# johannesulf/nautilus

Measured on AMD Instinct MI355X. Metric: effective posterior samples/sec + |dlogZ| vs analytic, 50-dim Gaussian, higher is better.
Workload: dtype f64

## Files before the change

include/nautilus_hip.h:

```cpp
#ifndef NAUTILUS_HIP_H
#define NAUTILUS_HIP_H

#include <stdint.h>

#ifdef __cplusplus
extern "C" {
#endif

#define NB_ABI_VERSION 6

typedef struct nb_bound nb_bound;
typedef struct nb_boundlist nb_boundlist;

typedef struct {
  int32_t n_ell;
  const int32_t* idx_ell;
  const double* c;
  const double* B;
  const double* B_inv;
  int32_t free_dims;
} nb_member_desc;

typedef struct {
  int32_t n_networks;
  const double* mean;
  const double* scale;
  const double* const* coefs;
  const double* const* intercepts;
} nb_mlp_desc;

typedef struct {
  nb_member_desc ellipsoid;
  const nb_mlp_desc* mlp;
  double score_predict_min;
  double radius2;
} nb_neural_desc;

typedef struct {
  int32_t n_dim;
  int32_t n_members;
  const nb_member_desc* members;
  const double* log_v_all;
  int32_t unit_cube;
  int32_t n_neural;
  const nb_neural_desc* neural;
  int32_t n_periodic;
  const int32_t* periodic;
  const double* centers;
} nb_bound_desc;

int nb_abi_version(void);
const char* nb_last_error(void);

int nb_bound_create(const nb_bound_desc* desc, nb_bound** out);
int nb_bound_destroy(nb_bound* bound);
int64_t nb_bound_nbytes(const nb_bound* bound);

int nb_boundlist_create(nb_bound* const* bounds, int32_t n, nb_boundlist** out);
int nb_boundlist_destroy(nb_boundlist* list);

int nb_contains(const nb_bound* bound, const double* x_dev, int64_t n,
                uint8_t* mask_dev, void* stream);

int nb_contains_any(const nb_boundlist* list, const double* x_dev, int64_t n,
                    uint8_t* mask_dev, void* stream);

int nb_first_containing(const nb_boundlist* list, const double* x_dev,
                        int64_t n, int32_t* idx_dev, void* stream);

int nb_member_count(const nb_bound* bound, const double* x_dev, int64_t n,
                    uint8_t* count_dev, void* stream);

int nb_neural_score(const nb_bound* bound, const double* x_dev, int64_t n,
                    double* out_dev, void* stream);

int nb_propose(const nb_bound* bound, uint64_t seed, uint64_t offset,
               int64_t n, double* x_dev, void* stream);

int nb_accept(const nb_bound* bound, uint64_t seed, uint64_t offset,
              const double* x_dev, int64_t n, uint8_t* flags_dev,
              void* stream);

int64_t nb_compact_scratch_bytes(int64_t n);
int nb_compact_rows(const double* x_dev, const uint8_t* flags_dev,
                    uint8_t mask, uint8_t flip, int64_t n, int32_t n_dim,
                    double* out_dev, int64_t* src_idx_dev, int64_t* counts_dev,
                    void* scratch_dev, void* stream);

int nb_shell_stats(const double* log_l_dev, int64_t n, double threshold,
                   double* out_dev, void* scratch_dev, void* stream);
int64_t nb_shell_stats_scratch_bytes(int64_t n);

int nb_live_append(const double* log_l_dev, int64_t n, const double* thr_dev,
                   double* pool_dev, int32_t* pool_n_dev, int32_t capacity,
                   int32_t* overflow_dev, void* stream);
int nb_live_select(const double* pool_dev, const int32_t* pool_n_dev,
                   int32_t capacity, int32_t k, double* pool_out_dev,
                   int32_t* pool_out_n_dev, double* thr_dev, double* stats_dev,
                   void* stream);
int nb_live_stats(const double* log_l_dev, int64_t n, const double* thr_dev,
                  double* out_dev, void* stream);

typedef struct nb_trainer nb_trainer;
int nb_trainer_create(int32_t n_dim, int32_t n_networks, int64_t n_rows,
                      const double* x_dev, const double* y_dev,
                      const double* const* coefs_host,
                      const double* const* intercepts_host,
                      nb_trainer** out);
int nb_trainer_create_fleet(int32_t n_dim, int32_t n_networks,
                            const int64_t* n_rows_of,
                            const double* const* x_dev_of,
                            const double* const* y_dev_of,
                            const double* const* coefs_host,
                            const double* const* intercepts_host,
                            nb_trainer** out);
#define NB_TRAIN_MAX_BATCH 4096
int nb_trainer_set_hparams(nb_trainer* t, double lr, double beta1,
                           double beta2, double epsilon, int32_t batch,
                           int32_t max_iter, int32_t n_iter_no_change,
                           double tol);
int nb_trainer_run(nb_trainer* t, const int32_t* perm_dev, int32_t n_epochs,
                   int32_t* status_host, void* stream);
int nb_trainer_run_fleet(nb_trainer* t, const int32_t* const* perm_dev_of,
                         int32_t n_epochs, int32_t* status_host, void* stream);
int nb_trainer_status(nb_trainer* t, int32_t* status_host, void* stream);
int nb_trainer_run_async(nb_trainer* t, const int32_t* const* perm_dev_of,
                         int32_t n_epochs, void* stream, int64_t* ticket);
int nb_trainer_wait(nb_trainer* t, int64_t ticket, int32_t* status_host);
int nb_host_shuffle_epochs(int32_t n_streams, uint32_t* const* key_of,
                           int32_t* pos, const int64_t* n_of, int32_t n_epochs,
                           int32_t* const* order_of, int32_t* const* out_of);
int nb_trainer_loss_curve(nb_trainer* t, int32_t net, double* out_host,
                          int32_t max_len);
int nb_trainer_weights(nb_trainer* t, int32_t net, double* const* coefs_host,
                       double* const* intercepts_host);
int nb_trainer_destroy(nb_trainer* t);

int nb_philox_uniform(uint64_t seed, uint64_t offset, uint32_t block,
                      uint32_t tag, int64_t n, double* u_dev, void* stream);

int nb_set_eval_counters(uint64_t* counters_dev);

int nb_mfma_f64_peak(int32_t iters, double* tflops_host);

int64_t nb_mvee_weights_work_doubles(int64_t n, int32_t n_dim,
                                     int32_t n_batch);
int nb_mvee_weights(const double* x_dev, int64_t n, int32_t n_dim,
                    int32_t n_max, int32_t n_batch, double* u_dev,
                    double* work_dev, void* stream);

int64_t nb_whiten_work_doubles(int64_t n, int32_t n_dim);
int nb_whiten(const double* x_dev, int64_t n, int32_t n_dim, double* xw_dev,
              double* mean_dev, double* sd_dev, double* w_dev,
              double* work_dev, void* stream);

int64_t nb_mvee_work_doubles(int32_t n_problems, int64_t n_points_max,
                             int32_t n_dim, int32_t n_batch);
int nb_mvee_khachiyan(int32_t n_problems, const double* const* xs_dev,
                      const int64_t* n_points, int32_t n_dim, int32_t n_max,
                      int32_t n_batch, double* const* u_dev, double* work_dev,
                      void* stream);

int64_t nb_moments_work_doubles(int64_t n, int32_t n_dim);
int nb_weighted_moments(const double* x_dev, const double* w_dev, int64_t n,
                        int32_t n_dim, double scale, double* out_dev,
                        double* work_dev, void* stream);

int64_t nb_quadform_work_doubles(void);
int nb_quadform_max(const double* x_dev, int64_t n, int32_t n_dim,
                    const double* p_dev, double* out_dev, double* work_dev,
                    void* stream);

int nb_ellipsoid_transform(const nb_bound* bound, const double* x_dev,
                           int64_t n, double* y_dev, void* stream);

int nb_standardize(const double* x_dev, int64_t n, int32_t n_dim,
                   double* mean_dev, double* scale_dev, double* out_dev,
                   void* stream);

int nb_prior_transform(const double* u_dev, int64_t n, int32_t n_dim,
                       const uint8_t* kind, const double* loc,
                       const double* scale, double* out_dev, void* stream);

typedef struct nb_prior_table nb_prior_table;
#define NB_PRIOR_ROW_MAJOR 0
#define NB_PRIOR_COLUMN_MAJOR 1
#define NB_PRIOR_LOG_SPACE 35.0
#define NB_PRIOR_TRUNCNORM_MAX 1e150
int nb_prior_table_create(int32_t n_dim, const uint8_t* kind,
                          const double* loc, const double* scale,
                          const double* shape0, const double* shape1,
                          int32_t n_keys, const int32_t* key_column,
                          const double* key_value, nb_prior_table** out);
int nb_prior_table_destroy(nb_prior_table* table);
int nb_prior_table_transform(const nb_prior_table* table, const double* u_dev,
                             int64_t n, int32_t layout, double* out_dev,
                             void* stream);

int nb_loglike_rosenbrock(const double* u_dev, int64_t n, int32_t n_dim,
                          double lo, double hi, double a, double* out_dev,
                          void* stream);
int nb_loglike_funnel(const double* u_dev, int64_t n, int32_t n_dim, double mu,
                      double sigma0, double k, double c, double* out_dev,
                      void* stream);


int64_t nb_list_eval_work_bytes(const nb_boundlist* list, int64_t n);
int nb_list_eval(const nb_boundlist* list, int32_t mode, const double* x_dev,
                 int64_t n, uint8_t* st_dev, int32_t* first_dev, void* work_dev,
                 int64_t work_bytes, void* stream);
int64_t nb_accept_staged_work_bytes(const nb_bound* bound, int64_t n);
int nb_accept_staged(const nb_bound* bound, uint64_t seed, uint64_t offset,
                     const double* x_dev, int64_t n, uint8_t* flags_dev,
                     void* work_dev, int64_t work_bytes, int64_t* totals_offset,
                     void* stream);
int nb_neural_score_rows(const nb_bound* bound, int32_t m, int32_t recentre,
                         const double* x_dev, const int64_t* idx_dev,
                         int64_t n, double* out_dev, void* stream);

int64_t nb_gmm_out_doubles(int32_t n_dim);
int64_t nb_gmm_scratch_doubles(int64_t n, int32_t n_dim);
int64_t nb_gmm_work_doubles(int64_t n, int32_t n_dim, int32_t n_init);
int64_t nb_gmm_logp_offset(int32_t n_dim);
int nb_gmm_fit(const double* x_dev, int64_t n, int32_t n_dim, int32_t n_init,
               uint64_t seed, double tol, double reg_covar, int32_t max_iter,
               const int32_t* init_labels_dev, double* out_dev,
               double* scratch_dev, void* stream);
int nb_gmm_set_max_wgs(int32_t max_wgs);

int nb_phase_shift(double* x_dev, int64_t n, int32_t n_dim, int32_t n_periodic,
                   const int32_t* periodic, const double* centers,
                   int32_t inverse, void* stream);

#define NB_COMM_ID_BYTES 128
typedef struct nb_comm nb_comm;
int nb_comm_unique_id(uint8_t* id_out );
int nb_comm_init(int32_t rank, int32_t n_ranks, const uint8_t* id,
                 nb_comm** out);
int nb_comm_destroy(nb_comm* comm);
uint64_t nb_comm_rank_key(uint64_t seed, int32_t rank);
int nb_comm_allgather_f64(nb_comm* comm, const double* send_dev, int64_t count,
                          double* recv_dev ,
                          void* stream);
int nb_comm_allreduce_i64(nb_comm* comm, int64_t* buf_dev ,
                          int64_t count, void* stream);

int nb_ellipsoid_contains_stream(const nb_bound* bound, const double* x_dev,
                                 int64_t n, uint8_t* mask_dev, void* stream);

#ifdef __cplusplus
}
#endif
#endif
```

nautilus_amd/_lib.py:

```python

import ctypes as C
import os

_HERE = os.path.dirname(os.path.abspath(__file__))
LIB_PATH = os.environ.get('NAUTILUS_HIP_LIB') or os.path.join(
    _HERE, 'lib', 'libnautilus_hip.so')

ABI_VERSION = 6

c_double_p = C.POINTER(C.c_double)
c_int32_p = C.POINTER(C.c_int32)


class MemberDesc(C.Structure):
    _fields_ = [('n_ell', C.c_int32), ('idx_ell', c_int32_p),
                ('c', c_double_p), ('B', c_double_p), ('B_inv', c_double_p),
                ('free_dims', C.c_int32)]


class MlpDesc(C.Structure):
    _fields_ = [('n_networks', C.c_int32), ('mean', c_double_p),
                ('scale', c_double_p), ('coefs', C.POINTER(c_double_p)),
                ('intercepts', C.POINTER(c_double_p))]


class NeuralDesc(C.Structure):
    _fields_ = [('ellipsoid', MemberDesc), ('mlp', C.POINTER(MlpDesc)),
                ('score_predict_min', C.c_double), ('radius2', C.c_double)]


class BoundDesc(C.Structure):
    _fields_ = [('n_dim', C.c_int32), ('n_members', C.c_int32),
                ('members', C.POINTER(MemberDesc)), ('log_v_all', c_double_p),
                ('unit_cube', C.c_int32), ('n_neural', C.c_int32),
                ('neural', C.POINTER(NeuralDesc)),
                ('n_periodic', C.c_int32), ('periodic', c_int32_p),
                ('centers', c_double_p)]


_SIGNATURES = {
    'nb_abi_version': (C.c_int, []),
    'nb_last_error': (C.c_char_p, []),
    'nb_bound_create': (C.c_int, [C.POINTER(BoundDesc),
                                  C.POINTER(C.c_void_p)]),
    'nb_bound_destroy': (C.c_int, [C.c_void_p]),
    'nb_bound_nbytes': (C.c_int64, [C.c_void_p]),
    'nb_boundlist_create': (C.c_int, [C.POINTER(C.c_void_p), C.c_int32,
                                      C.POINTER(C.c_void_p)]),
    'nb_boundlist_destroy': (C.c_int, [C.c_void_p]),
    'nb_contains': (C.c_int, [C.c_void_p, C.c_void_p, C.c_int64, C.c_void_p,
                              C.c_void_p]),
    'nb_contains_any': (C.c_int, [C.c_void_p, C.c_void_p, C.c_int64,
                                  C.c_void_p, C.c_void_p]),
    'nb_first_containing': (C.c_int, [C.c_void_p, C.c_void_p, C.c_int64,
                                      C.c_void_p, C.c_void_p]),
    'nb_member_count': (C.c_int, [C.c_void_p, C.c_void_p, C.c_int64,
                                  C.c_void_p, C.c_void_p]),
    'nb_neural_score': (C.c_int, [C.c_void_p, C.c_void_p, C.c_int64,
                                  C.c_void_p, C.c_void_p]),
    'nb_propose': (C.c_int, [C.c_void_p, C.c_uint64, C.c_uint64, C.c_int64,
                             C.c_void_p, C.c_void_p]),
    'nb_accept': (C.c_int, [C.c_void_p, C.c_uint64, C.c_uint64, C.c_void_p,
                            C.c_int64, C.c_void_p, C.c_void_p]),
    'nb_compact_scratch_bytes': (C.c_int64, [C.c_int64]),
    'nb_compact_rows': (C.c_int, [C.c_void_p, C.c_void_p, C.c_uint8,
                                  C.c_uint8, C.c_int64, C.c_int32, C.c_void_p,
                                  C.c_void_p, C.c_void_p, C.c_void_p,
                                  C.c_void_p]),
    'nb_shell_stats': (C.c_int, [C.c_void_p, C.c_int64, C.c_double,
                                 C.c_void_p, C.c_void_p, C.c_void_p]),
    'nb_shell_stats_scratch_bytes': (C.c_int64, [C.c_int64]),
    'nb_trainer_create': (C.c_int, [C.c_int32, C.c_int32, C.c_int64,
                                    C.c_void_p, C.c_void_p,
                                    C.POINTER(c_double_p),
                                    C.POINTER(c_double_p),
                                    C.POINTER(C.c_void_p)]),
    'nb_trainer_create_fleet': (C.c_int, [C.c_int32, C.c_int32, C.c_void_p,
                                          C.c_void_p, C.c_void_p, C.c_void_p,
                                          C.c_void_p, C.c_void_p]),
    'nb_trainer_run_fleet': (C.c_int, [C.c_void_p, C.c_void_p, C.c_int32,
                                       C.c_void_p, C.c_void_p]),
    'nb_trainer_set_hparams': (C.c_int, [C.c_void_p, C.c_double, C.c_double,
                                         C.c_double, C.c_double, C.c_int32,
                                         C.c_int32, C.c_int32, C.c_double]),
    'nb_trainer_run': (C.c_int, [C.c_void_p, C.c_void_p, C.c_int32,
                                 c_int32_p, C.c_void_p]),
    'nb_trainer_status': (C.c_int, [C.c_void_p, c_int32_p, C.c_void_p]),
    'nb_trainer_run_async': (C.c_int, [C.c_void_p, C.c_void_p, C.c_int32,
                                       C.c_void_p, C.POINTER(C.c_int64)]),
    'nb_trainer_wait': (C.c_int, [C.c_void_p, C.c_int64, c_int32_p]),
    'nb_host_shuffle_epochs': (C.c_int, [C.c_int32, C.c_void_p, c_int32_p,
                                         C.c_void_p, C.c_int32, C.c_void_p,
                                         C.c_void_p]),
    'nb_trainer_loss_curve': (C.c_int, [C.c_void_p, C.c_int32, c_double_p,
                                        C.c_int32]),
    'nb_trainer_weights': (C.c_int, [C.c_void_p, C.c_int32,
                                     C.POINTER(c_double_p),
                                     C.POINTER(c_double_p)]),
    'nb_trainer_destroy': (C.c_int, [C.c_void_p]),
    'nb_philox_uniform': (C.c_int, [C.c_uint64, C.c_uint64, C.c_uint32,
                                    C.c_uint32, C.c_int64, C.c_void_p,
                                    C.c_void_p]),
    'nb_set_eval_counters': (C.c_int, [C.c_void_p]),
    'nb_mfma_f64_peak': (C.c_int, [C.c_int32, c_double_p]),
    'nb_mvee_weights': (C.c_int, [C.c_void_p, C.c_int64, C.c_int32, C.c_int32,
                                  C.c_int32, C.c_void_p, C.c_void_p,
                                  C.c_void_p]),
    'nb_mvee_weights_work_doubles': (C.c_int64, [C.c_int64, C.c_int32,
                                                 C.c_int32]),
    'nb_mvee_work_doubles': (C.c_int64, [C.c_int32, C.c_int64, C.c_int32,
                                         C.c_int32]),
    'nb_mvee_khachiyan': (C.c_int, [C.c_int32, C.POINTER(C.c_void_p),
                                    C.POINTER(C.c_int64), C.c_int32,
                                    C.c_int32, C.c_int32,
                                    C.POINTER(C.c_void_p), C.c_void_p,
                                    C.c_void_p]),
    'nb_whiten_work_doubles': (C.c_int64, [C.c_int64, C.c_int32]),
    'nb_whiten': (C.c_int, [C.c_void_p, C.c_int64, C.c_int32, C.c_void_p,
                            C.c_void_p, C.c_void_p, C.c_void_p, C.c_void_p,
                            C.c_void_p]),
    'nb_moments_work_doubles': (C.c_int64, [C.c_int64, C.c_int32]),
    'nb_weighted_moments': (C.c_int, [C.c_void_p, C.c_void_p, C.c_int64,
                                      C.c_int32, C.c_double, C.c_void_p,
                                      C.c_void_p, C.c_void_p]),
    'nb_quadform_work_doubles': (C.c_int64, []),
    'nb_quadform_max': (C.c_int, [C.c_void_p, C.c_int64, C.c_int32,
                                  C.c_void_p, C.c_void_p, C.c_void_p,
                                  C.c_void_p]),
    'nb_ellipsoid_transform': (C.c_int, [C.c_void_p, C.c_void_p, C.c_int64,
                                         C.c_void_p, C.c_void_p]),
    'nb_standardize': (C.c_int, [C.c_void_p, C.c_int64, C.c_int32, C.c_void_p,
                                 C.c_void_p, C.c_void_p, C.c_void_p]),
    'nb_prior_transform': (C.c_int, [C.c_void_p, C.c_int64, C.c_int32,
                                     C.c_void_p, c_double_p, c_double_p,
                                     C.c_void_p, C.c_void_p]),
    'nb_prior_table_create': (C.c_int, [C.c_int32, C.c_void_p, c_double_p,
                                        c_double_p, c_double_p, c_double_p,
                                        C.c_int32, c_int32_p, c_double_p,
                                        C.POINTER(C.c_void_p)]),
    'nb_prior_table_destroy': (C.c_int, [C.c_void_p]),
    'nb_prior_table_transform': (C.c_int, [C.c_void_p, C.c_void_p, C.c_int64,
                                           C.c_int32, C.c_void_p, C.c_void_p]),
    'nb_loglike_rosenbrock': (C.c_int, [C.c_void_p, C.c_int64, C.c_int32,
                                        C.c_double, C.c_double, C.c_double,
                                        C.c_void_p, C.c_void_p]),
    'nb_loglike_funnel': (C.c_int, [C.c_void_p, C.c_int64, C.c_int32,
                                    C.c_double, C.c_double, C.c_double,
                                    C.c_double, C.c_void_p, C.c_void_p]),
    'nb_live_append': (C.c_int, [C.c_void_p, C.c_int64, C.c_void_p,
                                 C.c_void_p, C.c_void_p, C.c_int32,
                                 C.c_void_p, C.c_void_p]),
    'nb_live_select': (C.c_int, [C.c_void_p, C.c_void_p, C.c_int32, C.c_int32,
                                 C.c_void_p, C.c_void_p, C.c_void_p,
                                 C.c_void_p, C.c_void_p]),
    'nb_live_stats': (C.c_int, [C.c_void_p, C.c_int64, C.c_void_p,
                                C.c_void_p, C.c_void_p]),
    'nb_comm_unique_id': (C.c_int, [C.c_void_p]),
    'nb_comm_init': (C.c_int, [C.c_int32, C.c_int32, C.c_void_p,
                               C.POINTER(C.c_void_p)]),
    'nb_comm_destroy': (C.c_int, [C.c_void_p]),
    'nb_comm_rank_key': (C.c_uint64, [C.c_uint64, C.c_int32]),
    'nb_comm_allgather_f64': (C.c_int, [C.c_void_p, C.c_void_p, C.c_int64,
                                        C.c_void_p, C.c_void_p]),
    'nb_comm_allreduce_i64': (C.c_int, [C.c_void_p, C.c_void_p, C.c_int64,
                                        C.c_void_p]),
    'nb_list_eval_work_bytes': (C.c_int64, [C.c_void_p, C.c_int64]),
    'nb_list_eval': (C.c_int, [C.c_void_p, C.c_int32, C.c_void_p, C.c_int64,
                               C.c_void_p, C.c_void_p, C.c_void_p, C.c_int64,
                               C.c_void_p]),
    'nb_accept_staged_work_bytes': (C.c_int64, [C.c_void_p, C.c_int64]),
    'nb_accept_staged': (C.c_int, [C.c_void_p, C.c_uint64, C.c_uint64,
                                   C.c_void_p, C.c_int64, C.c_void_p,
                                   C.c_void_p, C.c_int64,
                                   C.POINTER(C.c_int64), C.c_void_p]),
    'nb_neural_score_rows': (C.c_int, [C.c_void_p, C.c_int32, C.c_int32,
                                       C.c_void_p, C.c_void_p, C.c_int64,
                                       C.c_void_p, C.c_void_p]),
    'nb_gmm_out_doubles': (C.c_int64, [C.c_int32]),
    'nb_gmm_scratch_doubles': (C.c_int64, [C.c_int64, C.c_int32]),
    'nb_gmm_work_doubles': (C.c_int64, [C.c_int64, C.c_int32, C.c_int32]),
    'nb_gmm_logp_offset': (C.c_int64, [C.c_int32]),
    'nb_gmm_fit': (C.c_int, [C.c_void_p, C.c_int64, C.c_int32, C.c_int32,
                             C.c_uint64, C.c_double, C.c_double, C.c_int32,
                             C.c_void_p, C.c_void_p, C.c_void_p, C.c_void_p]),
    'nb_gmm_set_max_wgs': (C.c_int, [C.c_int32]),
    'nb_phase_shift': (C.c_int, [C.c_void_p, C.c_int64, C.c_int32, C.c_int32,
                                 c_int32_p, c_double_p, C.c_int32,
                                 C.c_void_p]),
    'nb_ellipsoid_contains_stream': (C.c_int, [C.c_void_p, C.c_void_p,
                                               C.c_int64, C.c_void_p,
                                               C.c_void_p]),
}

_lib = None


def load():
    global _lib
    if _lib is not None:
        return _lib
    try:
        import torch
    except ImportError:
        pass
    if not os.path.exists(LIB_PATH):
        raise RuntimeError(
            'nautilus_amd: HIP library %s not found; run `make` (hipcc, '
            'gfx950).  There is no CPU fallback.' % LIB_PATH)
    lib = C.CDLL(LIB_PATH)
    for name, (res, args) in _SIGNATURES.items():
        fn = getattr(lib, name)
        fn.restype = res
        fn.argtypes = args
    if lib.nb_abi_version() != ABI_VERSION:
        raise RuntimeError(
            'nautilus_amd: %s has ABI version %d, this package binds version '
            '%d (rebuild with `make`)' % (LIB_PATH, lib.nb_abi_version(),
                                          ABI_VERSION))
    _lib = lib
    return lib


def exported_symbols():
    return sorted(_SIGNATURES)


ERR_ARG, ERR_HIP, ERR_UNSUPPORTED = 1, 2, 3


class NativeError(RuntimeError):

    def __init__(self, code, message):
        super().__init__('nautilus_hip: ' + message)
        self.code = code


def check(status):
    if status != 0:
        raise NativeError(status, load().nb_last_error().decode(
            'utf-8', 'replace'))
```

nautilus_amd/csrc/nb_api.hip:

```cpp
#include "nb_common.h"
#include "../../include/nautilus_hip.h"

#include <cmath>
#include <cstdarg>
#include <cstdio>
#include <csignal>
#include <cstring>
#include <ctime>
#include <execinfo.h>
#include <limits>
#include <unistd.h>
#include <string>
#include <vector>

bool nb_eval_fast_eligible(int n_dim, int K, int M, int E, bool sample);
int nb_launch_eval_fast(const double* blob_dev, int n_dim, bool sample, int m,
                        int recentre, const double* x, const long long* idx,
                        long long n,
                        unsigned char* out_u8, double* out_f64,
                        unsigned long long seed, unsigned long long offset,
                        hipStream_t stream);
int nb_launch_cand(int dt, int n_dim, const double* const* blobs_dev,
                   const int* group_base_dev, int nb, int n_groups, int b_off,
                   int g_off, int accumulate, int mode, const double* x,
                   long long n, unsigned char* st, int* first, int* work,
                   unsigned long long seed, unsigned long long offset,
                   int** dense_out, int** totals_out, long long* n_pad_out,
                   hipStream_t stream);
long long nb_cand_work_bytes(int dt, int mode, long long n, int n_groups);
int nb_launch_eval_fast_batch(const double* blob0_dev, int n_dim, int recentre,
                              const double* x, const void* groups_dev,
                              int n_groups, const int* totals_dev,
                              const int* dense_dev, long long n_pad,
                              long long n_upper, int out_mode,
                              unsigned char* st, int* first,
                              hipStream_t stream);
int nb_launch_eval(int dt, const double* const* blobs_dev, int nb, int mode,
                   const double* x, long long n, unsigned char* out_u8,
                   int* out_i32, double* out_f64, unsigned long long seed,
                   unsigned long long offset, hipStream_t stream);
void nb_eval_set_counters(unsigned long long* dev);
int nb_launch_draw(const double* blob_dev, int n_dim, unsigned long long seed,
                   unsigned long long offset, long long n, double* x_out,
                   hipStream_t stream);
long long nb_compact_chunks(long long n);
int nb_launch_compact(const double* x, const unsigned char* flags,
                      unsigned char mask, unsigned char flip, long long n,
                      int n_dim, double* out,
                      long long* src_idx, long long* counts,
                      long long* chunk_counts, hipStream_t stream);
int nb_lse_blocks(long long n);
int nb_launch_shell_stats(const double* log_l, long long n, double threshold,
                          double* out, double* partial, hipStream_t stream);
int nb_launch_philox(unsigned long long seed, unsigned long long offset,
                     unsigned block, unsigned tag, long long n, double* u,
                     hipStream_t stream);
int nb_run_mfma_peak(int iters, double* tflops);
int nb_launch_mvee_batch(int n_problems, const double* const* xs,
                         const long long* n, int d, int n_max, int n_batch,
                         double* const* u, double* work, hipStream_t stream);
long long nb_mvee_work_doubles_impl(int n_problems, long long n_max, int d,
                                    int n_batch);
int nb_launch_moments(const double* x, const double* w, long long n, int d,
                      double scale, double* out, double* work,
                      hipStream_t stream);
long long nb_moments_work_doubles_impl(long long n, int d);
int nb_launch_quadform_max(const double* x, long long n, int d,
                           const double* p_dev, double* out, double* work,
                           hipStream_t stream);
long long nb_quadform_work_doubles_impl();
int nb_launch_live_append(const double* ll, long long n, const double* thr,
                          double* pool, int* pool_n, int cap, int* overflow,
                          hipStream_t stream);
int nb_launch_live_select(const double* pool, const int* pool_n, int cap,
                          int k, double* out, int* out_n, double* thr,
                          double* stats, hipStream_t stream);
int nb_launch_live_stats(const double* ll, long long n, const double* thr,
                         double* out, hipStream_t stream);
int nb_launch_rosenbrock(const double* u, long long n, int d, double lo,
                         double hi, double a, double* out, hipStream_t stream);
int nb_launch_funnel(const double* u, long long n, int d, double mu, double s0,
                     double k, double c, double* out, hipStream_t stream);
long long nb_whiten_work_doubles_impl(long long n, int d);
int nb_launch_whiten(const double* x, long long n, int d, double* xw,
                     double* mean, double* sd, double* w, double* work,
                     hipStream_t stream);
int nb_launch_transform(const double* ell_block, int dt, int n_dim,
                        const double* x, long long n, double* y,
                        hipStream_t stream);
int nb_launch_standardize(const double* x, long long n, int d, double* mean,
                          double* scale, double* out, hipStream_t stream);
int nb_launch_prior(const double* u, long long n, int d,
                    const unsigned char* kind, const double* loc,
                    const double* scale, double* out, hipStream_t stream);
int nb_launch_prior_table(const double* u, long long n, int d,
                          const double* par, const unsigned char* kind,
                          int n_keys, const int* key_column,
                          const double* key_value, int column_major,
                          int level, double* out, hipStream_t stream);
long long nb_gmm_out_stride_impl(int d);
long long nb_gmm_scratch_stride_impl(long long n, int d);
long long nb_gmm_work_doubles_impl(long long n, int d, int n_init);
long long nb_gmm_logp_offset_impl(long long n, int d);
int nb_gmm_set_cap_impl(int max_wgs);
int nb_launch_gmm(const double* x, long long n, int d, int n_init,
                  unsigned long long seed, double tol, double reg, int max_iter,
                  const int* init_labels, double* out, double* scratch,
                  hipStream_t stream);
int nb_launch_phase_shift(double* x, long long n, int n_dim, const double* s,
                          const unsigned char* on, int inverse,
                          hipStream_t stream);
int nb_launch_ell_stream(const double* cvec, const double* binv, int n_dim,
                         const double* x, long long n, unsigned char* mask,
                         hipStream_t stream);

static thread_local std::string g_error;

void nb_set_error(const char* fmt, ...) {
  char buf[1024];
  va_list ap;
  va_start(ap, fmt);
  vsnprintf(buf, sizeof buf, fmt, ap);
  va_end(ap);
  g_error = buf;
}

struct nb_bound {
  double* blob_dev = nullptr;
  const double** self_list_dev = nullptr;
  FastGroup* groups_dev = nullptr;
  int* group_base_dev = nullptr;
  int n_groups = 0;
  int64_t off_shift = 0, neural_stride = 0;
  int64_t n_doubles = 0;
  int n_dim = 0, dt = 0, K = 0, M = 0, E = 0;
  bool single_full_ellipsoid = false;
  int64_t off_stream = 0;
  int64_t off_members = 0, off_neural = 0;
};

static inline int64_t nb_hdr_host_off_members(const nb_bound* b) {
  return b->off_members;
}

struct nb_boundlist {
  const double** ptrs_dev = nullptr;
  int n = 0, dt = 0, n_dim = 0;
  int blocks_single = 0;
  FastGroup* groups_dev = nullptr;
  int* group_base_dev = nullptr;
  std::vector<int> group_base;
  int n_groups = 0;
  const double* blob0 = nullptr;
};

static void nb_append_groups(const nb_bound* b, int pos,
                             std::vector<FastGroup>& out) {
  if (b->E < 1) return;
  for (int m = 0; m < b->M; ++m) {
    FastGroup g;
    g.nb = b->blob_dev + b->off_neural + (int64_t)m * b->neural_stride;
    g.shift = b->off_shift != 0 ? b->blob_dev + b->off_shift : nullptr;
    g.E = b->E;
    g.b = pos;
    out.push_back(g);
  }
}

namespace {

const double INF = std::numeric_limits<double>::infinity();

inline void put_i64(std::vector<double>& buf, size_t at, int64_t v) {
  std::memcpy(&buf[at], &v, sizeof v);
}

inline int slot_of_feature(int f) {
  const int j = f >> 3, r = f & 7;
  const int lg = r >> 1, o = r & 1;
  return 4 * (2 * j + o) + lg;
}

bool fill_ell_block(std::vector<double>& buf, size_t at, int n_dim, int dt,
                    const nb_member_desc& m, bool is_neural) {
  const int dp = 16 * dt;
  if (m.n_ell < 0 || m.n_ell > n_dim) {
    nb_set_error("member n_ell=%d out of range for n_dim=%d", m.n_ell, n_dim);
    return false;
  }
  put_i64(buf, at, m.n_ell);
  double* lo = &buf[at + 2];
  double* hi = lo + dp;
  double* c = hi + dp;
  double* tiles = c + dp;
  std::vector<int> idx(m.n_ell);
  std::vector<char> is_ell(n_dim, 0);
  for (int i = 0; i < m.n_ell; ++i) {
    idx[i] = m.idx_ell ? m.idx_ell[i] : i;
    if (idx[i] < 0 || idx[i] >= n_dim || (i > 0 && idx[i] <= idx[i - 1])) {
      nb_set_error("idx_ell must be strictly increasing within [0, n_dim)");
      return false;
    }
    is_ell[idx[i]] = 1;
  }
  bool any_box = false;
  for (int f = 0; f < dp; ++f) {
    const bool boxed = f < n_dim && !is_ell[f] && !m.free_dims && !is_neural;
    const int sl = slot_of_feature(f);
    lo[sl] = boxed ? 0.0 : -INF;
    hi[sl] = boxed ? 1.0 : INF;
    c[sl] = 0.0;
    any_box |= boxed;
  }
  put_i64(buf, at + 1, any_box ? 1 : 0);
  for (int i = 0; i < m.n_ell; ++i) c[slot_of_feature(idx[i])] = m.c[i];
  for (int i = 0; i < m.n_ell; ++i) {
    for (int j = 0; j < m.n_ell; ++j) {
      const double v = m.B_inv[(size_t)i * m.n_ell + j];
      if (j > i) {
        if (v != 0.0) {
          nb_set_error("B_inv must be lower triangular (basic.py:308-309)");
          return false;
        }
        continue;
      }
      const int h = idx[i], k = idx[j];
      const int sl = slot_of_feature(k);
      const int ks = sl >> 2, lgk = sl & 3;
      tiles[((size_t)(ks >> 2) * dt + (h >> 4)) * NB_TILE + (ks & 3) * 64 +
            lgk * 16 + (h & 15)] = v;
    }
  }
  return true;
}

void put_weight(double* tiles, int ht_n, int k, int h, double v) {
  tiles[((size_t)(k >> 4) * ht_n + (h >> 4)) * NB_TILE + (k & 15) * 16 +
        (h & 15)] = v;
}

void fill_net(double* net, int n_dim, int kt1, const double* const* coefs,
              const double* const* intercepts) {
  double* w1 = net;
  double* w2 = w1 + (size_t)kt1 * NB_HT1 * NB_TILE;
  double* w3 = w2 + (size_t)NB_HT1 * NB_HT2 * NB_TILE;
  double* w4 = w3 + (size_t)NB_HT2 * NB_HT3 * NB_TILE;
  for (int k = 0; k < n_dim; ++k)
    for (int h = 0; h < NB_H1; ++h)
      put_weight(w1, NB_HT1, k, h, coefs[0][(size_t)k * NB_H1 + h]);
  for (int h = 0; h < NB_H1; ++h)
    put_weight(w1, NB_HT1, n_dim, h, intercepts[0][h]);
  for (int k = 0; k < NB_H1; ++k)
    for (int h = 0; h < NB_H2; ++h)
      put_weight(w2, NB_HT2, k, h, coefs[1][(size_t)k * NB_H2 + h]);
  for (int h = 0; h < NB_H2; ++h)
    put_weight(w2, NB_HT2, NB_H1, h, intercepts[1][h]);
  for (int k = 0; k < NB_H2; ++k)
    for (int h = 0; h < NB_H3; ++h)
      put_weight(w3, NB_HT3, k, h, coefs[2][(size_t)k * NB_H3 + h]);
  for (int h = 0; h < NB_H3; ++h)
    put_weight(w3, NB_HT3, NB_H2, h, intercepts[2][h]);
  for (int k = 0; k < NB_H3; ++k) put_weight(w4, 1, k, 0, coefs[3][k]);
  put_weight(w4, 1, NB_H3, 0, intercepts[3][0]);
}

inline hipStream_t as_stream(void* s) { return (hipStream_t)s; }

}

extern "C" {

int nb_abi_version(void) { return NB_ABI_VERSION; }

const char* nb_last_error(void) { return g_error.c_str(); }

int nb_bound_create(const nb_bound_desc* d, nb_bound** out) {
  if (d == nullptr || out == nullptr) {
    nb_set_error("null argument");
    return NB_ERR_ARG;
  }
  const int n_dim = d->n_dim;
  if (n_dim < 1 || n_dim > 16 * NB_MAX_DT) {
    nb_set_error("n_dim=%d unsupported (1..%d)", n_dim, 16 * NB_MAX_DT);
    return NB_ERR_UNSUPPORTED;
  }
  const int dt = (n_dim + 15) / 16, dp = 16 * dt;
  const int K = d->n_members, M = d->n_neural;
  if (K < 0 || M < 0 || (K > 0 && d->members == nullptr) ||
      (M > 0 && d->neural == nullptr)) {
    nb_set_error("inconsistent member / neural counts");
    return NB_ERR_ARG;
  }
  int E = 0;
  for (int m = 0; m < M; ++m) {
    const int e = d->neural[m].mlp ? d->neural[m].mlp->n_networks : 0;
    if (m > 0 && e != E) {
      nb_set_error("all neural bounds must have the same number of networks");
      return NB_ERR_ARG;
    }
    E = e;
    if (d->neural[m].ellipsoid.n_ell != n_dim) {
      nb_set_error("NeuralBound ellipsoid must span all dimensions");
      return NB_ERR_ARG;
    }
  }
  const int kt1 = (n_dim + 1 + 15) / 16;
  const int64_t ell_size = nb_ell_block_size(dt);
  const int64_t net_stride = (int64_t)nb_net_tiles(kt1) * NB_TILE;
  const int64_t neural_stride = ell_size + 2 + 2 * dp + (int64_t)E * net_stride;
  const int64_t draw_stride = 2 + 4 * dp + (int64_t)dp * (dp + 1) / 2 + 16;

  int64_t off = NB_HDR;
  const int64_t off_cdf = off; off += ((K > 0 ? K : 1) + 1) / 2 * 2;
  const int64_t off_ulo = off; off += dp;
  const int64_t off_uhi = off; off += dp;
  const int64_t off_members = off; off += (int64_t)K * ell_size;
  const int64_t off_neural = off; off += (int64_t)M * neural_stride;
  const int64_t off_draw = off; off += (int64_t)K * draw_stride;
  const bool single_full = (K == 1 && M == 0 && !d->unit_cube &&
                            d->members[0].n_ell == n_dim);
  const int64_t off_stream = off;
  if (single_full) off += dp + (int64_t)dt * (dt + 1) / 2 * NB_TILE;
  if (d->n_periodic < 0 || d->n_periodic > n_dim ||
      (d->n_periodic > 0 && (d->periodic == nullptr || d->centers == nullptr))) {
    nb_set_error("bad periodic description");
    return NB_ERR_ARG;
  }
  const int64_t off_shift = off;
  if (d->n_periodic > 0) off += 2 * dp;
  const int64_t total = off;

  std::vector<double> buf((size_t)total, 0.0);
  put_i64(buf, NB_H_NDIM, n_dim);
  put_i64(buf, NB_H_DT, dt);
  put_i64(buf, NB_H_K, K);
  put_i64(buf, NB_H_USECUBE, d->unit_cube ? 1 : 0);
  put_i64(buf, NB_H_M, M);
  put_i64(buf, NB_H_E, E);
  put_i64(buf, NB_H_OFF_CDF, off_cdf);
  put_i64(buf, NB_H_OFF_ULO, off_ulo);
  put_i64(buf, NB_H_OFF_UHI, off_uhi);
  put_i64(buf, NB_H_OFF_MEMBERS, off_members);
  put_i64(buf, NB_H_ELL_STRIDE, ell_size);
  put_i64(buf, NB_H_OFF_NEURAL, off_neural);
  put_i64(buf, NB_H_NEURAL_STRIDE, neural_stride);
  put_i64(buf, NB_H_OFF_DRAW, off_draw);
  put_i64(buf, NB_H_DRAW_STRIDE, draw_stride);
  put_i64(buf, NB_H_NET_STRIDE, net_stride);
  put_i64(buf, NB_H_KT1, kt1);
  put_i64(buf, NB_H_TOTAL, total);
  put_i64(buf, NB_H_OFF_STREAM, single_full ? off_stream : 0);
  put_i64(buf, NB_H_OFF_SHIFT, d->n_periodic > 0 ? off_shift : 0);
  for (int i = 0; i < d->n_periodic; ++i) {
    const int f = d->periodic[i];
    if (f < 0 || f >= n_dim) {
      nb_set_error("periodic index %d out of range", f);
      return NB_ERR_ARG;
    }
    buf[off_shift + slot_of_feature(f)] = -d->centers[i] + 0.5;
    buf[off_shift + dp + slot_of_feature(f)] = 1.0;
  }
  if (single_full) {
    const nb_member_desc& md = d->members[0];
    for (int i = 0; i < n_dim; ++i) buf[off_stream + i] = md.c[i];
    double* st = &buf[off_stream + dp];
    for (int ht = 0; ht < dt; ++ht)
      for (int kt = 0; kt <= ht; ++kt)
        for (int s4 = 0; s4 < 4; ++s4)
          for (int lg = 0; lg < 4; ++lg)
            for (int li = 0; li < 16; ++li) {
              const int k = 16 * kt + 8 * (s4 >> 1) + 2 * lg + (s4 & 1);
              const int h = 16 * ht + li;
              double v = 0.0;
              if (h < n_dim && k < n_dim && k <= h)
                v = md.B_inv[(size_t)h * n_dim + k];
              st[((size_t)(ht * (ht + 1)) / 2 + kt) * NB_TILE + s4 * 64 +
                 lg * 16 + li] = v;
            }
  }

  if (K > 0) {
    double mx = -INF;
    for (int m = 0; m < K; ++m)
      mx = std::fmax(mx, d->log_v_all ? d->log_v_all[m] : 0.0);
    std::vector<double> p(K);
    double sum = 0.0;
    for (int m = 0; m < K; ++m) {
      p[m] = std::exp((d->log_v_all ? d->log_v_all[m] : 0.0) - mx);
      sum += p[m];
    }
    double run = 0.0;
    for (int m = 0; m < K; ++m) {
      run += p[m] / sum;
      buf[off_cdf + m] = run;
    }
    buf[off_cdf + K - 1] = 1.0;
  }
  for (int f = 0; f < dp; ++f) {
    const bool boxed = d->unit_cube && f < n_dim;
    buf[off_ulo + slot_of_feature(f)] = boxed ? 0.0 : -INF;
    buf[off_uhi + slot_of_feature(f)] = boxed ? 1.0 : INF;
  }

  for (int m = 0; m < K; ++m) {
    const nb_member_desc& md = d->members[m];
    if (!fill_ell_block(buf, off_members + m * ell_size, n_dim, dt, md, false))
      return NB_ERR_ARG;
    const size_t at = off_draw + m * draw_stride;
    std::vector<char> is_ell(n_dim, 0);
    for (int i = 0; i < md.n_ell; ++i)
      is_ell[md.idx_ell ? md.idx_ell[i] : i] = 1;
    int nc = 0;
    for (int f = 0; f < n_dim; ++f) {
      if (!is_ell[f] && !md.free_dims) {
        put_i64(buf, at + 2 + dp + nc, f);
        ++nc;
      }
    }
    put_i64(buf, at, md.n_ell);
    put_i64(buf, at + 1, nc);
    {
      int cube_slot = md.n_ell;
      for (int f = 0; f < n_dim; ++f)
        if (!is_ell[f]) put_i64(buf, at + 2 + 2 * dp + f, cube_slot++);
    }
    for (int i = 0; i < md.n_ell; ++i) {
      const int f = md.idx_ell ? md.idx_ell[i] : i;
      put_i64(buf, at + 2 + i, f);
      put_i64(buf, at + 2 + 2 * dp + f, i);
      buf[at + 2 + 3 * dp + i] = md.c[i];
      for (int j = 0; j <= i; ++j)
        buf[at + 2 + 4 * dp + (size_t)i * (i + 1) / 2 + j] =
            md.B[(size_t)i * md.n_ell + j];
    }
  }

  for (int m = 0; m < M; ++m) {
    const nb_neural_desc& nd = d->neural[m];
    const size_t at = off_neural + m * neural_stride;
    if (!fill_ell_block(buf, at, n_dim, dt, nd.ellipsoid, true))
      return NB_ERR_ARG;
    buf[at + ell_size] = nd.score_predict_min - 1e-9;
    {
      double r2 = nd.radius2;
      if (!(r2 > 0.0)) {
        const int n = nd.ellipsoid.n_ell;
        const double* B = nd.ellipsoid.B;
        double fro = 0.0, ger = 0.0;
        for (int i = 0; i < n * n; ++i) fro += B[i] * B[i];
        for (int i = 0; i < n; ++i) {
          double rowsum = 0.0;
          for (int j = 0; j < n; ++j) {
            double aij = 0.0;
            for (int k = 0; k < n; ++k) aij += B[i * n + k] * B[j * n + k];
            rowsum += std::fabs(aij);
          }
          ger = std::fmax(ger, rowsum);
        }
        r2 = std::fmin(fro, ger) * (1.0 + 1e-9);
      }
      buf[at + 1] = r2;
    }
    double* mean = &buf[at + ell_size + 2];
    double* scale = mean + dp;
    for (int f = 0; f < dp; ++f) { mean[f] = 0.0; scale[f] = 1.0; }
    if (nd.mlp != nullptr) {
      for (int f = 0; f < n_dim; ++f) {
        mean[f] = nd.mlp->mean[f];
        scale[f] = 1.0 / nd.mlp->scale[f];
      }
      for (int e = 0; e < E; ++e)
        fill_net(scale + dp + (size_t)e * net_stride, n_dim, kt1,
                 nd.mlp->coefs + 4 * e, nd.mlp->intercepts + 4 * e);
    }
  }

  nb_bound* b = new nb_bound();
  b->n_doubles = total;
  b->n_dim = n_dim; b->dt = dt; b->K = K; b->M = M; b->E = E;
  b->single_full_ellipsoid = single_full;
  b->off_stream = off_stream;
  b->off_members = off_members;
  b->off_neural = off_neural;
  b->off_shift = nb_hdr(buf.data(), NB_H_OFF_SHIFT);
  b->neural_stride = nb_hdr(buf.data(), NB_H_NEURAL_STRIDE);
  constexpr size_t SLACK = 512;
  hipError_t e = hipMalloc((void**)&b->blob_dev,
                           ((size_t)total + SLACK) * sizeof(double));
  if (e == hipSuccess)
    e = hipMemset(b->blob_dev + total, 0, SLACK * sizeof(double));
  if (e == hipSuccess)
    e = hipMemcpy(b->blob_dev, buf.data(), (size_t)total * sizeof(double),
                  hipMemcpyHostToDevice);
  if (e == hipSuccess) e = hipMalloc((void**)&b->self_list_dev, sizeof(double*));
  if (e == hipSuccess)
    e = hipMemcpy(b->self_list_dev, &b->blob_dev, sizeof(double*),
                  hipMemcpyHostToDevice);
  if (e == hipSuccess) {
    std::vector<FastGroup> groups;
    nb_append_groups(b, 0, groups);
    b->n_groups = (int)groups.size();
    const int base[2] = {0, b->n_groups};
    e = hipMalloc((void**)&b->group_base_dev, sizeof base);
    if (e == hipSuccess)
      e = hipMemcpy(b->group_base_dev, base, sizeof base,
                    hipMemcpyHostToDevice);
    if (e == hipSuccess && b->n_groups > 0) {
      e = hipMalloc((void**)&b->groups_dev, groups.size() * sizeof(FastGroup));
      if (e == hipSuccess)
        e = hipMemcpy(b->groups_dev, groups.data(),
                      groups.size() * sizeof(FastGroup), hipMemcpyHostToDevice);
    }
  }
  if (e != hipSuccess) {
    nb_set_error("bound upload failed: %s", hipGetErrorString(e));
    nb_bound_destroy(b);
    return NB_ERR_HIP;
  }
  *out = b;
  return NB_OK;
}

int nb_bound_destroy(nb_bound* b) {
  if (b == nullptr) return NB_OK;
  if (b->blob_dev) (void)hipFree(b->blob_dev);
  if (b->self_list_dev) (void)hipFree(b->self_list_dev);
  if (b->groups_dev) (void)hipFree(b->groups_dev);
  if (b->group_base_dev) (void)hipFree(b->group_base_dev);
  delete b;
  return NB_OK;
}

int64_t nb_bound_nbytes(const nb_bound* b) {
  return b ? b->n_doubles * (int64_t)sizeof(double) : 0;
}

int nb_boundlist_create(nb_bound* const* bounds, int32_t n,
                        nb_boundlist** out) {
  if (n < 0 || (n > 0 && bounds == nullptr) || out == nullptr) {
    nb_set_error("bad bound list");
    return NB_ERR_ARG;
  }
  nb_boundlist* l = new nb_boundlist();
  l->n = n;
  std::vector<const double*> ptrs(n);
  for (int i = 0; i < n; ++i) {
    if (i > 0 && bounds[i]->n_dim != bounds[0]->n_dim) {
      nb_set_error("bounds of a list must share n_dim");
      delete l;
      return NB_ERR_ARG;
    }
    ptrs[i] = bounds[i]->blob_dev;
  }
  if (n > 0) {
    l->dt = bounds[0]->dt;
    l->n_dim = bounds[0]->n_dim;
    l->blob0 = bounds[0]->blob_dev;
    if (n == 1) l->blocks_single = bounds[0]->K + bounds[0]->M;
    hipError_t e = hipMalloc((void**)&l->ptrs_dev, n * sizeof(double*));
    if (e == hipSuccess)
      e = hipMemcpy(l->ptrs_dev, ptrs.data(), n * sizeof(double*),
                    hipMemcpyHostToDevice);
    std::vector<FastGroup> groups;
    l->group_base.assign(1, 0);
    for (int i = 0; i < n; ++i) {
      nb_append_groups(bounds[i], i, groups);
      l->group_base.push_back((int)groups.size());
    }
    l->n_groups = (int)groups.size();
    if (e == hipSuccess)
      e = hipMalloc((void**)&l->group_base_dev, (n + 1) * sizeof(int));
    if (e == hipSuccess)
      e = hipMemcpy(l->group_base_dev, l->group_base.data(),
                    (n + 1) * sizeof(int), hipMemcpyHostToDevice);
    if (e == hipSuccess && l->n_groups > 0) {
      e = hipMalloc((void**)&l->groups_dev, groups.size() * sizeof(FastGroup));
      if (e == hipSuccess)
        e = hipMemcpy(l->groups_dev, groups.data(),
                      groups.size() * sizeof(FastGroup), hipMemcpyHostToDevice);
    }
    if (e != hipSuccess) {
      nb_set_error("bound list upload failed: %s", hipGetErrorString(e));
      nb_boundlist_destroy(l);
      return NB_ERR_HIP;
    }
  }
  *out = l;
  return NB_OK;
}

int nb_boundlist_destroy(nb_boundlist* l) {
  if (l == nullptr) return NB_OK;
  if (l->ptrs_dev) (void)hipFree(l->ptrs_dev);
  if (l->groups_dev) (void)hipFree(l->groups_dev);
  if (l->group_base_dev) (void)hipFree(l->group_base_dev);
  delete l;
  return NB_OK;
}

int nb_contains(const nb_bound* b, const double* x, int64_t n, uint8_t* mask,
                void* stream) {
  return nb_launch_eval(b->dt, b->self_list_dev, 1, 0, x, n, mask, nullptr,
                        nullptr, 0, 0, as_stream(stream));
}

int nb_contains_any(const nb_boundlist* l, const double* x, int64_t n,
                    uint8_t* mask, void* stream) {
  if (l->n == 0) {
    NB_HIP_CHECK(hipMemsetAsync(mask, 0, (size_t)n, as_stream(stream)));
    return NB_OK;
  }
  return nb_launch_eval(l->dt, l->ptrs_dev, l->n, 0, x, n, mask, nullptr,
                        nullptr, 0, 0, as_stream(stream));
}

int nb_first_containing(const nb_boundlist* l, const double* x, int64_t n,
                        int32_t* idx, void* stream) {
  if (l->n == 0) {
    NB_HIP_CHECK(hipMemsetAsync(idx, 0xFF, (size_t)n * 4, as_stream(stream)));
    return NB_OK;
  }
  return nb_launch_eval(l->dt, l->ptrs_dev, l->n, 1, x, n, nullptr, idx,
                        nullptr, 0, 0, as_stream(stream));
}

int nb_member_count(const nb_bound* b, const double* x, int64_t n,
                    uint8_t* count, void* stream) {
  return nb_launch_eval(b->dt, b->self_list_dev, 1, 3, x, n, count, nullptr,
                        nullptr, 0, 0, as_stream(stream));
}

int nb_neural_score(const nb_bound* b, const double* x, int64_t n, double* out,
                    void* stream) {
  if (b->M < 1) {
    nb_set_error("bound has no neural bound");
    return NB_ERR_ARG;
  }
#ifndef NB_NO_FAST_EVAL
  if (nb_eval_fast_eligible(b->n_dim, b->K, b->M, b->E, false))
    return nb_launch_eval_fast(b->blob_dev, b->n_dim, false, 0, 0, x, nullptr, n,
                               nullptr, out, 0, 0, as_stream(stream));
#endif
  return nb_launch_eval(b->dt, b->self_list_dev, 1, 4, x, n, nullptr, nullptr,
                        out, 0, 0, as_stream(stream));
}

static void nb_abort_trace(int sig) {
  void* frames[64];
  const int n = backtrace(frames, 64);
  const char msg[] = "[nautilus_hip] fatal signal, native backtrace:\n";
  (void)!write(2, msg, sizeof msg - 1);
  backtrace_symbols_fd(frames, n, 2);
  signal(sig, SIG_DFL);
  raise(sig);
}

__attribute__((constructor)) static void nb_install_abort_trace(void) {
  if (getenv("NB_ABORT_TRACE") == nullptr) return;
  signal(SIGABRT, nb_abort_trace);
  signal(SIGSEGV, nb_abort_trace);
}

static int nb_slice_groups() {
  const char* e = getenv("NB_LIST_SLICE_GROUPS");
  const int v = e != nullptr ? atoi(e) : 1024;
  return v < 1 ? 1 : (v > 1024 ? 1024 : v);
}
#define NB_SLICE_GROUPS nb_slice_groups()

int64_t nb_list_eval_work_bytes(const nb_boundlist* l, int64_t n) {
  const int g = l->n_groups < NB_SLICE_GROUPS ? l->n_groups : NB_SLICE_GROUPS;
  int most = 0;
  for (int i = 0; i < l->n; ++i) {
    const int k = l->group_base[i + 1] - l->group_base[i];
    most = k > most ? k : most;
  }
  return nb_cand_work_bytes(l->dt, 0, n, (g > most ? g : most) + 1);
}

int64_t nb_accept_staged_work_bytes(const nb_bound* b, int64_t n) {
  return nb_cand_work_bytes(b->dt, 2, n, b->n_groups + 1);
}

static int nb_stage_two(const double* blob0, int n_dim, int recentre,
                        const double* x, const FastGroup* groups, int n_groups,
                        int* totals, int* dense, long long n_pad, long long n,
                        int mode, uint8_t* st, int32_t* first,
                        hipStream_t stream) {
  if (n_groups == 0) return NB_OK;
  return nb_launch_eval_fast_batch(blob0, n_dim, recentre, x, groups, n_groups,
                                   totals, dense, n_pad,
                                   (long long)n * (n_groups < 8 ? n_groups : 8),
                                   mode, st, first, stream);
}

int nb_list_eval(const nb_boundlist* l, int32_t mode, const double* x,
                 int64_t n, uint8_t* st, int32_t* first, void* work,
                 int64_t work_bytes, void* stream) {
  if (mode != 0 && mode != 1) {
    nb_set_error("nb_list_eval: mode must be 0 (any) or 1 (first)");
    return NB_ERR_ARG;
  }
  if (mode == 1 && first == nullptr) {
    nb_set_error("nb_list_eval: mode 1 needs the `first` output");
    return NB_ERR_ARG;
  }
  if (n <= 0) return NB_OK;
  if (l->n == 0) {
    NB_HIP_CHECK(hipMemsetAsync(st, 0, (size_t)n, as_stream(stream)));
    if (first != nullptr)
      NB_HIP_CHECK(hipMemsetD32Async((hipDeviceptr_t)first, 0x7fffffff,
                                     (size_t)n, as_stream(stream)));
    return NB_OK;
  }
  if (work_bytes < nb_list_eval_work_bytes(l, n)) {
    nb_set_error("nb_list_eval: work space of %lld bytes, need %lld",
                 (long long)work_bytes,
                 (long long)nb_list_eval_work_bytes(l, n));
    return NB_ERR_ARG;
  }
  int b0 = 0;
  while (b0 < l->n) {
    int b1 = b0 + 1;
    while (b1 < l->n && l->group_base[b1 + 1] - l->group_base[b0] <=
                            NB_SLICE_GROUPS)
      ++b1;
    const int g0 = l->group_base[b0], ng = l->group_base[b1] - g0;
    int *dense = nullptr, *totals = nullptr;
    long long n_pad = 0;
    int rc = nb_launch_cand(l->dt, l->n_dim, l->ptrs_dev + b0, l->group_base_dev + b0,
                            b1 - b0, ng, b0, g0, b0 > 0 ? 1 : 0, mode, x, n,
                            st, first, (int*)work, 0, 0, &dense, &totals,
                            &n_pad, as_stream(stream));
    if (rc != NB_OK) return rc;
    rc = nb_stage_two(l->blob0, l->n_dim, 1, x, l->groups_dev + g0, ng, totals,
                      dense, n_pad, n, mode, st, first, as_stream(stream));
    if (rc != NB_OK) return rc;
    b0 = b1;
  }
  return NB_OK;
}

int nb_accept_staged(const nb_bound* b, uint64_t seed, uint64_t offset,
                     const double* x, int64_t n, uint8_t* flags, void* work,
                     int64_t work_bytes, int64_t* totals_offset, void* stream) {
  if (n <= 0) return NB_OK;
  if (work_bytes < nb_accept_staged_work_bytes(b, n)) {
    nb_set_error("nb_accept_staged: work space of %lld bytes, need %lld",
                 (long long)work_bytes,
                 (long long)nb_accept_staged_work_bytes(b, n));
    return NB_ERR_ARG;
  }
  int *dense = nullptr, *totals = nullptr;
  long long n_pad = 0;
  static const bool timing = getenv("NB_STAGE_TIMING") != nullptr;
  static hipEvent_t ev[3][3];
  static double host_us[3][4];
  static int ev_calls = 0;
  hipEvent_t* e = nullptr;
  double* hu = nullptr;
  auto now_us = []() {
    timespec ts;
    clock_gettime(CLOCK_MONOTONIC, &ts);
    return ts.tv_sec * 1e6 + ts.tv_nsec * 1e-3;
  };
  if (timing) {
    if (ev_calls == 0)
      for (int i = 0; i < 9; ++i) (void)hipEventCreate(&ev[i / 3][i % 3]);
    if (ev_calls > 1) {
      hipEvent_t* p = ev[(ev_calls - 2) % 3];
      hipEvent_t* q = ev[(ev_calls - 1) % 3];
      const double* h = host_us[(ev_calls - 2) % 3];
      const double* hq = host_us[(ev_calls - 1) % 3];
      float t_geo = 0.f, t_emu = 0.f, t_gap = 0.f;
      (void)hipEventSynchronize(q[0]);
      (void)hipEventElapsedTime(&t_geo, p[0], p[1]);
      (void)hipEventElapsedTime(&t_emu, p[1], p[2]);
      (void)hipEventElapsedTime(&t_gap, p[2], q[0]);
      fprintf(stderr, "[stage] call %d: device: candidates + compaction %.3f "
              "ms, batched scores %.3f ms, then idle until the next call's "
              "first event %.3f ms; host: stage-one launches %.0f us, "
              "stage-two launch %.0f us, until the next call %.0f us\n",
              ev_calls - 2, t_geo, t_emu, t_gap, h[1] - h[0], h[2] - h[1],
              hq[0] - h[2]);
    }
    e = ev[ev_calls % 3];
    hu = host_us[ev_calls % 3];
    ++ev_calls;
    hu[0] = now_us();
    (void)hipEventRecord(e[0], as_stream(stream));
  }
  int rc = nb_launch_cand(b->dt, b->n_dim, b->self_list_dev, b->group_base_dev, 1,
                          b->n_groups, 0, 0, 0, 2, x, n, flags, nullptr,
                          (int*)work, seed, offset, &dense, &totals, &n_pad,
                          as_stream(stream));
  if (rc != NB_OK) return rc;
  if (e != nullptr) {
    (void)hipEventRecord(e[1], as_stream(stream));
    hu[1] = now_us();
  }
  if (totals_offset != nullptr)
    *totals_offset = (int64_t)((char*)totals - (char*)work);
  rc = nb_stage_two(b->blob_dev, b->n_dim, 0, x, b->groups_dev, b->n_groups,
                    totals, dense, n_pad, n, 2, flags, nullptr,
                    as_stream(stream));
  if (e != nullptr) {
    (void)hipEventRecord(e[2], as_stream(stream));
    hu[2] = now_us();
  }
  return rc;
}

int nb_neural_score_rows(const nb_bound* b, int32_t m, int32_t recentre,
                         const double* x, const int64_t* idx, int64_t n,
                         double* out, void* stream) {
  if (m < 0 || m >= b->M || b->E < 1) {
    nb_set_error("nb_neural_score_rows: neural bound %d of %d (E = %d)", m,
                 b->M, b->E);
    return NB_ERR_ARG;
  }
  return nb_launch_eval_fast(b->blob_dev, b->n_dim, false, m, recentre, x,
                             (const long long*)idx, n, nullptr, out, 0, 0,
                             as_stream(stream));
}

int nb_propose(const nb_bound* b, uint64_t seed, uint64_t offset, int64_t n,
               double* x, void* stream) {
  if (b->K < 1) {
    nb_set_error("bound has no outer members to draw from");
    return NB_ERR_ARG;
  }
  return nb_launch_draw(b->blob_dev, b->n_dim, seed, offset, n, x,
                        as_stream(stream));
}

int nb_accept(const nb_bound* b, uint64_t seed, uint64_t offset,
              const double* x, int64_t n, uint8_t* flags, void* stream) {
#ifndef NB_NO_FAST_EVAL
  if (nb_eval_fast_eligible(b->n_dim, b->K, b->M, b->E, true))
    return nb_launch_eval_fast(b->blob_dev, b->n_dim, true, 0, 0, x, nullptr, n,
                               flags, nullptr, seed, offset,
                               as_stream(stream));
#endif
  return nb_launch_eval(b->dt, b->self_list_dev, 1, 2, x, n, flags, nullptr,
                        nullptr, seed, offset, as_stream(stream));
}

int64_t nb_compact_scratch_bytes(int64_t n) {
  return (nb_compact_chunks(n) * 2 + 2) * (int64_t)sizeof(long long);
}

int nb_compact_rows(const double* x, const uint8_t* flags, uint8_t mask,
                    uint8_t flip, int64_t n, int32_t n_dim, double* out,
                    int64_t* src_idx, int64_t* counts, void* scratch,
                    void* stream) {
  return nb_launch_compact(x, flags, mask, flip, n, n_dim, out,
                           (long long*)src_idx, (long long*)counts,
                           (long long*)scratch, as_stream(stream));
}

int64_t nb_shell_stats_scratch_bytes(int64_t n) {
  return (int64_t)nb_lse_blocks(n) * 4 * sizeof(double);
}

int nb_shell_stats(const double* log_l, int64_t n, double threshold,
                   double* out, void* scratch, void* stream) {
  return nb_launch_shell_stats(log_l, n, threshold, out, (double*)scratch,
                               as_stream(stream));
}

int nb_philox_uniform(uint64_t seed, uint64_t offset, uint32_t block,
                      uint32_t tag, int64_t n, double* u, void* stream) {
  return nb_launch_philox(seed, offset, block, tag, n, u, as_stream(stream));
}

int nb_set_eval_counters(uint64_t* counters_dev) {
  nb_eval_set_counters((unsigned long long*)counters_dev);
  return NB_OK;
}

int nb_mfma_f64_peak(int32_t iters, double* tflops) {
  return nb_run_mfma_peak(iters, tflops);
}

int64_t nb_mvee_work_doubles(int32_t n_problems, int64_t n_points_max,
                             int32_t n_dim, int32_t n_batch) {
  return nb_mvee_work_doubles_impl(n_problems, n_points_max, n_dim, n_batch);
}

int nb_mvee_khachiyan(int32_t n_problems, const double* const* xs,
                      const int64_t* n_points, int32_t n_dim, int32_t n_max,
                      int32_t n_batch, double* const* u, double* work,
                      void* stream) {
  if (n_problems < 1 || xs == nullptr || n_points == nullptr || u == nullptr ||
      work == nullptr) {
    nb_set_error("null argument");
    return NB_ERR_ARG;
  }
  std::vector<long long> n(n_points, n_points + n_problems);
  return nb_launch_mvee_batch(n_problems, xs, n.data(), n_dim, n_max, n_batch,
                              u, work, as_stream(stream));
}

int64_t nb_whiten_work_doubles(int64_t n, int32_t n_dim) {
  return nb_whiten_work_doubles_impl(n, n_dim);
}

int nb_whiten(const double* x, int64_t n, int32_t n_dim, double* xw,
              double* mean, double* sd, double* w, double* work,
              void* stream) {
  if (x == nullptr || xw == nullptr || mean == nullptr || sd == nullptr ||
      w == nullptr || work == nullptr) {
    nb_set_error("null argument");
    return NB_ERR_ARG;
  }
  return nb_launch_whiten(x, n, n_dim, xw, mean, sd, w, work,
                          as_stream(stream));
}

int64_t nb_mvee_weights_work_doubles(int64_t n, int32_t n_dim,
                                     int32_t n_batch) {
  return 2 * 16 * NB_MAX_DT + (int64_t)n_dim * n_dim + n * n_dim + 4 +
         nb_whiten_work_doubles_impl(n, n_dim) +
         nb_mvee_work_doubles_impl(1, n, n_dim, n_batch);
}

int nb_mvee_weights(const double* x, int64_t n, int32_t n_dim, int32_t n_max,
                    int32_t n_batch, double* u, double* work, void* stream) {
  if (x == nullptr || u == nullptr || work == nullptr) {
    nb_set_error("null argument");
    return NB_ERR_ARG;
  }
  if (n_dim < 1 || n_dim > 16 * NB_MAX_DT) {
    nb_set_error("device MVEE supports n_dim <= 128 (got %d)", n_dim);
    return NB_ERR_UNSUPPORTED;
  }
  double* mean = work;
  double* scale = work + 16 * NB_MAX_DT;
  double* wmat = scale + 16 * NB_MAX_DT;
  double* xw = wmat + (((int64_t)n_dim * n_dim + 1) & ~(int64_t)1);
  double* wh = xw + ((n * n_dim + 1) & ~(int64_t)1);
  double* rest = wh + nb_whiten_work_doubles_impl(n, n_dim);
  int rc = nb_launch_whiten(x, n, n_dim, xw, mean, scale, wmat, wh,
                            as_stream(stream));
  if (rc != NB_OK) return rc;
  const double* xw_c = xw;
  long long nn = n;
  return nb_launch_mvee_batch(1, &xw_c, &nn, n_dim, n_max, n_batch, &u, rest,
                              as_stream(stream));
}

int64_t nb_moments_work_doubles(int64_t n, int32_t n_dim) {
  return nb_moments_work_doubles_impl(n, n_dim);
}

int nb_weighted_moments(const double* x, const double* w, int64_t n,
                        int32_t n_dim, double scale, double* out, double* work,
                        void* stream) {
  if (x == nullptr || out == nullptr || work == nullptr) {
    nb_set_error("null argument");
    return NB_ERR_ARG;
  }
  return nb_launch_moments(x, w, n, n_dim, scale, out, work,
                           as_stream(stream));
}

int64_t nb_quadform_work_doubles(void) {
  return nb_quadform_work_doubles_impl();
}

int nb_quadform_max(const double* x, int64_t n, int32_t n_dim,
                    const double* p_dev, double* out, double* work,
                    void* stream) {
  if (x == nullptr || p_dev == nullptr || out == nullptr || work == nullptr) {
    nb_set_error("null argument");
    return NB_ERR_ARG;
  }
  return nb_launch_quadform_max(x, n, n_dim, p_dev, out, work,
                                as_stream(stream));
}

int nb_ellipsoid_transform(const nb_bound* b, const double* x, int64_t n,
                           double* y, void* stream) {
  const double* blk = nullptr;
  if (b->single_full_ellipsoid)
    blk = b->blob_dev + nb_hdr_host_off_members(b);
  else if (b->K == 0 && b->M >= 1)
    blk = b->blob_dev + b->off_neural;
  if (blk == nullptr) {
    nb_set_error("nb_ellipsoid_transform needs an Ellipsoid or a NeuralBound");
    return NB_ERR_ARG;
  }
  return nb_launch_transform(blk, b->dt, b->n_dim, x, n, y, as_stream(stream));
}

int nb_standardize(const double* x, int64_t n, int32_t n_dim, double* mean,
                   double* scale, double* out, void* stream) {
  if (x == nullptr || mean == nullptr || scale == nullptr) {
    nb_set_error("null argument");
    return NB_ERR_ARG;
  }
  return nb_launch_standardize(x, n, n_dim, mean, scale, out,
                               as_stream(stream));
}

int nb_prior_transform(const double* u, int64_t n, int32_t n_dim,
                       const uint8_t* kind, const double* loc,
                       const double* scale, double* out, void* stream) {
  if (n_dim < 1 || n_dim > 16 * NB_MAX_DT || kind == nullptr ||
      loc == nullptr || scale == nullptr || (n > 0 && (!u || !out))) {
    nb_set_error("bad prior transform arguments");
    return NB_ERR_ARG;
  }
  for (int j = 0; j < n_dim; ++j)
    if (kind[j] > 1) {
      nb_set_error("prior kind %d of parameter %d is not supported", kind[j], j);
      return NB_ERR_UNSUPPORTED;
    }
  return nb_launch_prior(u, n, n_dim, kind, loc, scale, out, as_stream(stream));
}

struct nb_prior_table {
  double* dev = nullptr;
  int n_dim = 0, n_keys = 0;
  int level = 0;
  const double* par() const { return dev; }
  const double* key_value() const { return dev + NB_PRIOR_NPAR * (size_t)n_dim; }
  const int* key_column() const { return (const int*)(key_value() + n_keys); }
  const unsigned char* kind() const {
    return (const unsigned char*)(key_column() + n_keys);
  }
};

namespace {

long double pt_phi(double x) {
  return 0.5L * erfcl(-(long double)x / sqrtl(2.0L));
}

void pt_truncnorm_constants(double a, double b, double* out3) {
  const long double cdf_a = pt_phi(a), sf_b = pt_phi(-b);
  long double mass;
  if (a > 0.0) {
    mass = pt_phi(-a) - sf_b;
  } else if (b < 0.0) {
    mass = pt_phi(b) - cdf_a;
  } else {
    mass = 0.5L * (erfl((long double)b / sqrtl(2.0L)) +
                   erfl(-(long double)a / sqrtl(2.0L)));
  }
  out3[0] = (double)cdf_a;
  out3[1] = (double)sf_b;
  out3[2] = (double)mass;
}

long double pt_log_erfcx_tail(double x) {
  const long double y = (long double)x / sqrtl(2.0L);
  long double term = 1.0L, sum = 1.0L;
  for (int k = 1; k <= 12; ++k) {
    term *= -(long double)(2 * k - 1) / (2.0L * y * y);
    sum += term;
  }
  return logl(sum) - logl(y) - 0.5L * logl(acosl(-1.0L));
}

void pt_truncnorm_log_constants(double a, double b, double* out3) {
  const long double log_ea = pt_log_erfcx_tail(a);
  long double r0 = 0.0L, r1 = 1.0L;
  if (std::isfinite(b)) {
    const long double log_r0 = pt_log_erfcx_tail(b) - log_ea -
        0.5L * ((long double)b - a) * ((long double)b + a);
    r0 = expl(log_r0);
    r1 = -expm1l(log_r0);
  }
  out3[0] = (double)log_ea;
  out3[1] = (double)r0;
  out3[2] = (double)r1;
}

}

int nb_prior_table_create(int32_t n_dim, const uint8_t* kind,
                          const double* loc, const double* scale,
                          const double* shape0, const double* shape1,
                          int32_t n_keys, const int32_t* key_column,
                          const double* key_value, nb_prior_table** out) {
  if (out == nullptr || n_dim < 1 || n_dim > 16 * NB_MAX_DT || n_keys < 1 ||
      kind == nullptr || loc == nullptr || scale == nullptr ||
      shape0 == nullptr || shape1 == nullptr || key_column == nullptr ||
      key_value == nullptr) {
    nb_set_error("bad prior table arguments");
    return NB_ERR_ARG;
  }
  *out = nullptr;
  const size_t d = (size_t)n_dim;
  std::vector<double> par(NB_PRIOR_NPAR * d, 0.0);
  std::vector<unsigned char> kind_dev(kind, kind + d);
  for (int j = 0; j < n_dim; ++j) {
    const double a = shape0[j], b = shape1[j];
    if (kind[j] > 5) {
      nb_set_error("prior kind %d of parameter %d is not supported", kind[j], j);
      return NB_ERR_UNSUPPORTED;
    }
    if (!std::isfinite(loc[j]) || !(scale[j] > 0.0) ||
        !std::isfinite(scale[j])) {
      nb_set_error("parameter %d: loc must be finite and scale positive", j);
      return NB_ERR_ARG;
    }
    par[0 * d + j] = loc[j];
    par[1 * d + j] = scale[j];
    if (kind[j] == 2) {
      if (!(a > 0.0) || !(a < b) || !std::isfinite(b)) {
        nb_set_error("parameter %d: log-uniform needs 0 < a < b < inf", j);
        return NB_ERR_ARG;
      }
      par[2 * d + j] = std::log(a);
      par[3 * d + j] = std::log(b) - std::log(a);
    } else if (kind[j] == 3) {
      if (!(a > 0.0) || !std::isfinite(a)) {
        nb_set_error("parameter %d: log-normal needs a shape s > 0", j);
        return NB_ERR_ARG;
      }
      par[2 * d + j] = a;
    } else if (kind[j] == 5) {
      if (!(a < b)) {
        nb_set_error("parameter %d: truncated normal needs a < b", j);
        return NB_ERR_ARG;
      }
      if (a > NB_PRIOR_TRUNCNORM_MAX || b < -NB_PRIOR_TRUNCNORM_MAX) {
        nb_set_error("parameter %d: a truncated normal whose interval lies "
                     "more than %g standard deviations from the mean is not "
                     "supported", j, (double)NB_PRIOR_TRUNCNORM_MAX);
        return NB_ERR_UNSUPPORTED;
      }
      double c3[3];
      if (a > NB_PRIOR_LOG_SPACE || b < -NB_PRIOR_LOG_SPACE) {
        const double sign = a > 0.0 ? 1.0 : -1.0;
        const double lo = a > 0.0 ? a : -b, hi = a > 0.0 ? b : -a;
        kind_dev[j] = 6;
        par[2 * d + j] = lo;
        par[3 * d + j] = hi;
        pt_truncnorm_log_constants(lo, hi, c3);
        par[7 * d + j] = sign;
      } else {
        par[2 * d + j] = a;
        par[3 * d + j] = b;
        pt_truncnorm_constants(a, b, c3);
      }
      for (int t = 0; t < 3; ++t) par[(4 + t) * d + j] = c3[t];
    }
  }
  for (int k = 0; k < n_keys; ++k)
    if (key_column[k] < -1 || key_column[k] >= n_dim) {
      nb_set_error("key %d refers to column %d of %d", k, key_column[k], n_dim);
      return NB_ERR_ARG;
    }
  const size_t bytes = (NB_PRIOR_NPAR * d + (size_t)n_keys) * sizeof(double) +
                       (size_t)n_keys * sizeof(int) + d;
  std::vector<unsigned char> host(bytes);
  unsigned char* at = host.data();
  std::memcpy(at, par.data(), NB_PRIOR_NPAR * d * sizeof(double));
  at += NB_PRIOR_NPAR * d * sizeof(double);
  std::memcpy(at, key_value, (size_t)n_keys * sizeof(double));
  at += (size_t)n_keys * sizeof(double);
  std::memcpy(at, key_column, (size_t)n_keys * sizeof(int));
  at += (size_t)n_keys * sizeof(int);
  std::memcpy(at, kind_dev.data(), d);
  nb_prior_table* t = new nb_prior_table;
  t->n_dim = n_dim;
  t->n_keys = n_keys;
  for (int j = 0; j < n_dim; ++j) {
    const int need = kind_dev[j] == 6 ? 2 : (kind[j] != 0 && kind[j] != 2);
    if (need > t->level) t->level = need;
  }
  hipError_t e = hipMalloc((void**)&t->dev, bytes);
  if (e == hipSuccess)
    e = hipMemcpy(t->dev, host.data(), bytes, hipMemcpyHostToDevice);
  if (e != hipSuccess) {
    nb_set_error("prior table upload failed: %s", hipGetErrorString(e));
    if (t->dev != nullptr) (void)hipFree(t->dev);
    delete t;
    return NB_ERR_HIP;
  }
  *out = t;
  return NB_OK;
}

int nb_prior_table_destroy(nb_prior_table* table) {
  if (table == nullptr) return NB_OK;
  (void)hipFree(table->dev);
  delete table;
  return NB_OK;
}

int nb_prior_table_transform(const nb_prior_table* table, const double* u,
                             int64_t n, int32_t layout, double* out,
                             void* stream) {
  if (table == nullptr || (layout != NB_PRIOR_ROW_MAJOR &&
                           layout != NB_PRIOR_COLUMN_MAJOR) ||
      n < 0 || (n > 0 && (u == nullptr || out == nullptr))) {
    nb_set_error("bad prior transform arguments");
    return NB_ERR_ARG;
  }
  return nb_launch_prior_table(u, n, table->n_dim, table->par(), table->kind(),
                               table->n_keys, table->key_column(),
                               table->key_value(),
                               layout == NB_PRIOR_COLUMN_MAJOR, table->level,
                               out,
                               as_stream(stream));
}

int nb_loglike_rosenbrock(const double* u, int64_t n, int32_t n_dim, double lo,
                          double hi, double a, double* out, void* stream) {
  if (n_dim < 2 || (n > 0 && (u == nullptr || out == nullptr))) {
    nb_set_error("bad Rosenbrock likelihood arguments");
    return NB_ERR_ARG;
  }
  return nb_launch_rosenbrock(u, n, n_dim, lo, hi, a, out, as_stream(stream));
}

int nb_loglike_funnel(const double* u, int64_t n, int32_t n_dim, double mu,
                      double sigma0, double k, double c, double* out,
                      void* stream) {
  if (n_dim < 2 || !(sigma0 > 0.0) || !(c > 0.0) ||
      (n > 0 && (u == nullptr || out == nullptr))) {
    nb_set_error("bad funnel likelihood arguments");
    return NB_ERR_ARG;
  }
  return nb_launch_funnel(u, n, n_dim, mu, sigma0, k, c, out,
                          as_stream(stream));
}

int nb_live_append(const double* log_l, int64_t n, const double* thr,
                   double* pool, int32_t* pool_n, int32_t capacity,
                   int32_t* overflow, void* stream) {
  if (capacity < 1 || thr == nullptr || pool == nullptr || pool_n == nullptr ||
      overflow == nullptr || (n > 0 && log_l == nullptr)) {
    nb_set_error("bad live-pool arguments");
    return NB_ERR_ARG;
  }
  return nb_launch_live_append(log_l, n, thr, pool, pool_n, capacity, overflow,
                               as_stream(stream));
}

int nb_live_select(const double* pool, const int32_t* pool_n, int32_t capacity,
                   int32_t k, double* pool_out, int32_t* pool_out_n,
                   double* thr, double* stats, void* stream) {
  if (capacity < 1 || k < 1 || pool == nullptr || pool_n == nullptr ||
      pool_out == nullptr || pool_out_n == nullptr || thr == nullptr ||
      stats == nullptr) {
    nb_set_error("bad live-pool arguments");
    return NB_ERR_ARG;
  }
  return nb_launch_live_select(pool, pool_n, capacity, k, pool_out, pool_out_n,
                               thr, stats, as_stream(stream));
}

int nb_live_stats(const double* log_l, int64_t n, const double* thr,
                  double* out, void* stream) {
  if (thr == nullptr || out == nullptr || (n > 0 && log_l == nullptr)) {
    nb_set_error("null argument");
    return NB_ERR_ARG;
  }
  return nb_launch_live_stats(log_l, n, thr, out, as_stream(stream));
}

int64_t nb_gmm_out_doubles(int32_t n_dim) {
  return nb_gmm_out_stride_impl(n_dim);
}

int64_t nb_gmm_scratch_doubles(int64_t n, int32_t n_dim) {
  return nb_gmm_scratch_stride_impl(n, n_dim);
}

int64_t nb_gmm_work_doubles(int64_t n, int32_t n_dim, int32_t n_init) {
  return nb_gmm_work_doubles_impl(n, n_dim, n_init);
}

int nb_gmm_set_max_wgs(int32_t max_wgs) { return nb_gmm_set_cap_impl(max_wgs); }
int64_t nb_gmm_logp_offset(int32_t n_dim) {
  return nb_gmm_logp_offset_impl(2, n_dim);
}

int nb_gmm_fit(const double* x, int64_t n, int32_t n_dim, int32_t n_init,
               uint64_t seed, double tol, double reg_covar, int32_t max_iter,
               const int32_t* init_labels, double* out, double* scratch,
               void* stream) {
  if (x == nullptr || out == nullptr || scratch == nullptr) {
    nb_set_error("null argument");
    return NB_ERR_ARG;
  }
  return nb_launch_gmm(x, n, n_dim, n_init, seed, tol, reg_covar, max_iter,
                       init_labels, out, scratch, as_stream(stream));
}

int nb_phase_shift(double* x, int64_t n, int32_t n_dim, int32_t n_periodic,
                   const int32_t* periodic, const double* centers,
                   int32_t inverse, void* stream) {
  if (n_dim < 1 || n_dim > 16 * NB_MAX_DT || n_periodic < 0 ||
      (n_periodic > 0 && (periodic == nullptr || centers == nullptr))) {
    nb_set_error("bad phase shift arguments");
    return NB_ERR_ARG;
  }
  double s[16 * NB_MAX_DT] = {0.0};
  unsigned char on[16 * NB_MAX_DT] = {0};
  for (int i = 0; i < n_periodic; ++i) {
    if (periodic[i] < 0 || periodic[i] >= n_dim) {
      nb_set_error("periodic index %d out of range", periodic[i]);
      return NB_ERR_ARG;
    }
    s[periodic[i]] = -centers[i] + 0.5;
    on[periodic[i]] = 1;
  }
  if (n <= 0 || n_periodic == 0) return NB_OK;
  return nb_launch_phase_shift(x, n, n_dim, s, on, inverse, as_stream(stream));
}

int nb_ellipsoid_contains_stream(const nb_bound* b, const double* x, int64_t n,
                                 uint8_t* mask, void* stream) {
  if (!b->single_full_ellipsoid) {
    nb_set_error("nb_ellipsoid_contains_stream needs a single full ellipsoid");
    return NB_ERR_ARG;
  }
  const double* cvec = b->blob_dev + b->off_stream;
  return nb_launch_ell_stream(cvec, cvec + 16 * b->dt, b->n_dim, x, n, mask,
                              as_stream(stream));
}

}
```

nautilus_amd/csrc/nb_common.h:

```cpp
#pragma once

#include <hip/hip_runtime.h>
#include <stdint.h>

#define NB_WAVE 64
#define NB_MAX_DT 8
#define NB_H1 100
#define NB_H2 50
#define NB_H3 20
#define NB_HT1 7
#define NB_HT2 4
#define NB_HT3 2
#define NB_TILE 256
#define NB_PRIOR_NPAR 8

typedef double nb_d4 __attribute__((ext_vector_type(4)));
typedef double nb_d2u __attribute__((ext_vector_type(2), aligned(8)));

#if defined(__HIP_DEVICE_COMPILE__)
#define NB_G __attribute__((address_space(1)))
#else
#define NB_G
#endif
typedef NB_G double nb_gd;
typedef NB_G int nb_gi;

#define NB_HDR 32

enum {
  NB_H_NDIM = 0, NB_H_DT, NB_H_K, NB_H_USECUBE, NB_H_M, NB_H_E, NB_H_OFF_CDF,
  NB_H_OFF_ULO, NB_H_OFF_UHI, NB_H_OFF_MEMBERS, NB_H_ELL_STRIDE,
  NB_H_OFF_NEURAL, NB_H_NEURAL_STRIDE, NB_H_OFF_DRAW, NB_H_DRAW_STRIDE,
  NB_H_NET_STRIDE, NB_H_KT1, NB_H_TOTAL, NB_H_OFF_STREAM, NB_H_OFF_SHIFT
};

__host__ __device__ inline int64_t nb_hdr(const double* blob, int i) {
  return ((const int64_t*)blob)[i];
}

__host__ __device__ constexpr int nb_ell_block_size(int dt) {
  return 2 + 3 * dt * 16 + dt * dt * NB_TILE;
}
__host__ __device__ inline int nb_net_tiles(int kt1) {
  return kt1 * NB_HT1 + NB_HT1 * NB_HT2 + NB_HT2 * NB_HT3 + NB_HT3 * 1;
}

struct FastGroup {
  const double* nb;
  const double* shift;
  int E;
  int b;
};

#define NB_TAG_CTRL 0u
#define NB_TAG_NORMAL 1u
#define NB_TAG_CUBE 2u

struct nb_u4 { uint32_t x, y, z, w; };

__host__ __device__ inline nb_u4 nb_philox(uint32_t c0, uint32_t c1, uint32_t c2,
                                           uint32_t c3, uint32_t k0, uint32_t k1) {
#pragma unroll
  for (int r = 0; r < 10; ++r) {
    const uint64_t p0 = (uint64_t)0xD2511F53u * c0;
    const uint64_t p1 = (uint64_t)0xCD9E8D57u * c2;
    const uint32_t n0 = (uint32_t)(p1 >> 32) ^ c1 ^ k0;
    const uint32_t n1 = (uint32_t)p1;
    const uint32_t n2 = (uint32_t)(p0 >> 32) ^ c3 ^ k1;
    const uint32_t n3 = (uint32_t)p0;
    c0 = n0; c1 = n1; c2 = n2; c3 = n3;
    k0 += 0x9E3779B9u; k1 += 0xBB67AE85u;
  }
  nb_u4 o = {c0, c1, c2, c3};
  return o;
}

__host__ __device__ inline double nb_unit(uint32_t hi, uint32_t lo) {
  return ((double)(hi >> 5) * 67108864.0 + (double)(lo >> 6)) *
         (1.0 / 9007199254740992.0);
}

__host__ __device__ inline double nb_unit32(uint32_t w) {
  return ((double)w + 0.5) * (1.0 / 4294967296.0);
}

__host__ __device__ inline void nb_uniform_pair(uint64_t seed, uint64_t g,
                                                uint32_t block, uint32_t tag,
                                                double& u0, double& u1) {
  nb_u4 w = nb_philox((uint32_t)g, (uint32_t)(g >> 32), block, tag,
                      (uint32_t)seed, (uint32_t)(seed >> 32));
  u0 = nb_unit(w.x, w.y);
  u1 = nb_unit(w.z, w.w);
}

#define NB_OK 0
#define NB_ERR_ARG 1
#define NB_ERR_HIP 2
#define NB_ERR_UNSUPPORTED 3

void nb_set_error(const char* fmt, ...);

#define NB_HIP_CHECK(expr)                                                   \
  do {                                                                       \
    hipError_t _e = (expr);                                                  \
    if (_e != hipSuccess) {                                                  \
      nb_set_error("%s failed: %s (%s:%d)", #expr, hipGetErrorString(_e),    \
                   __FILE__, __LINE__);                                      \
      return NB_ERR_HIP;                                                     \
    }                                                                        \
  } while (0)
```

nautilus_amd/csrc/nb_eval_fast.hip:

```cpp
#include "nb_common.h"

#include <type_traits>

#include "nb_mlp.h"

namespace {

constexpr int FAST_MAX_GROUPS = 1024;

struct FastArgs {
  const double* blob;
  int sample;
  const nb_gd* x;
  const long long* idx;
  int m;
  int recentre;
  long long n;
  unsigned char* out_u8;
  double* out_f64;
  unsigned long long seed;
  unsigned long long offset;
  unsigned long long* counters;
  const FastGroup* groups;
  const int* totals;
  const int* dense;
  long long n_pad;
  int n_groups;
  int out_mode;
  unsigned char* st;
  int* first;
};

constexpr int FAST_B_DOUBLES =
    (NB_HT1 * NB_HT2 + NB_HT2 * NB_HT3 + NB_HT3) * NB_TILE;

typedef const void __attribute__((address_space(1))) * nbf_gptr;
typedef void __attribute__((address_space(3))) * nbf_lptr;

template <int DT, int T>
__device__ __forceinline__ void ell_eval_centre(
    const double* c, const double* tiles, int n_dim,
    const double (&xin)[T][4 * DT], int lane, int lg, double (&y)[T][4 * DT],
    double (&r2)[T]) {
  double d[T][4 * DT];
#pragma unroll
  for (int ks = 0; ks < 4 * DT; ++ks) {
    const double cv = c[4 * ks + lg];
#pragma unroll
    for (int t = 0; t < T; ++t) d[t][ks] = xin[t][ks] - cv;
  }
  double part[T];
#pragma unroll
  for (int t = 0; t < T; ++t) part[t] = 0.0;
  const int live = n_dim - 16 * (DT - 1);
  const bool small = DT > 1 && live >= 1 && live <= 4;
  const int lane4 = (lane >> 4) * 16 + (lane & 3);
#pragma unroll
  for (int ht = 0; ht < DT; ++ht) {
    if (ht == DT - 1 && small) {
      double r4[T];
#pragma unroll
      for (int t = 0; t < T; ++t) r4[t] = 0.0;
#pragma unroll
      for (int ks = 0; ks < 4 * (ht + 1) - 2; ++ks) {
        const int kt = ks >> 2, s = ks & 3;
        const double a =
            tiles[(ht * (ht + 1) / 2 + kt) * NB_TILE + s * 64 + lane4];
#pragma unroll
        for (int t = 0; t < T; ++t) r4[t] = NB_MFMA4(a, d[t][ks], r4[t]);
      }
#pragma unroll
      for (int t = 0; t < T; ++t) {
        y[t][4 * ht] = r4[t];
        y[t][4 * ht + 1] = y[t][4 * ht + 2] = y[t][4 * ht + 3] = 0.0;
        part[t] += r4[t] * r4[t];
      }
    } else if (16 * ht < n_dim) {
      nb_d4 acc[T];
#pragma unroll
      for (int t = 0; t < T; ++t) acc[t] = nb_d4{0.0, 0.0, 0.0, 0.0};
#pragma unroll
      for (int ks = 0; ks < 4 * (ht + 1); ++ks) {
        const int kt = ks >> 2, s = ks & 3;
        const double a =
            tiles[(ht * (ht + 1) / 2 + kt) * NB_TILE + s * 64 + lane];
#pragma unroll
        for (int t = 0; t < T; ++t) acc[t] = MFMA(a, d[t][ks], acc[t]);
      }
#pragma unroll
      for (int t = 0; t < T; ++t)
#pragma unroll
        for (int r = 0; r < 4; ++r) {
          y[t][4 * ht + r] = acc[t][r];
          part[t] += acc[t][r] * acc[t][r];
        }
    } else {
#pragma unroll
      for (int t = 0; t < T; ++t)
#pragma unroll
        for (int r = 0; r < 4; ++r) y[t][4 * ht + r] = 0.0;
    }
  }
#pragma unroll
  for (int t = 0; t < T; ++t) r2[t] = lane_group_sum(part[t]);
}

template <int DT, int T>
__device__ __forceinline__ void load_points_raw(
    const nb_gd* __restrict__ x, const long long (&row_of)[T], int n_dim,
    int lane, double2 (&raw)[T][2 * DT]) {
  int lg = lane >> 4;
  asm volatile("" : "+v"(lg));
  asm volatile("" : "+s"(x));
  if ((n_dim & 1) == 0) {
#pragma unroll
    for (int t = 0; t < T; ++t) {
      const nb_gd* row = x + row_of[t] * n_dim;
#pragma unroll
      for (int j = 0; j < 2 * DT; ++j) {
        const int f = 8 * j + 2 * lg;
        raw[t][j] = *(const NB_G double2*)(row + (f < n_dim ? f : n_dim - 2));
      }
    }
  } else {
#pragma unroll
    for (int t = 0; t < T; ++t) {
      const nb_gd* row = x + row_of[t] * n_dim;
#pragma unroll
      for (int j = 0; j < 2 * DT; ++j) {
        const int f = 8 * j + 2 * lg;
        raw[t][j].x = row[f < n_dim ? f : n_dim - 1];
        raw[t][j].y = row[f + 1 < n_dim ? f + 1 : n_dim - 1];
      }
    }
  }
}

template <int DT, int T>
__device__ __forceinline__ void points_from_raw(
    const double2 (&raw)[T][2 * DT], const bool (&valid)[T], int n_dim,
    int lg, double (&xin)[T][4 * DT]) {
#pragma unroll
  for (int t = 0; t < T; ++t)
#pragma unroll
    for (int j = 0; j < 2 * DT; ++j) {
      const int f = 8 * j + 2 * lg;
      xin[t][2 * j] = (valid[t] && f < n_dim) ? raw[t][j].x : 0.0;
      xin[t][2 * j + 1] = (valid[t] && f + 1 < n_dim) ? raw[t][j].y : 0.0;
    }
}

constexpr int FAST_REGION = 38 * NB_TILE;

template <int DT, int KT1, bool BATCH>
__global__ void __launch_bounds__(512) nb_eval_fast_kernel(FastArgs a) {
  constexpr int T = 1, NW = 8, DP = 16 * DT;
  constexpr int KS1 = 4 * KT1;
  constexpr bool TWO = KT1 * NB_HT1 * NB_TILE > FAST_REGION;
  constexpr int KA = TWO ? (KT1 + 1) / 2 : KT1;
  constexpr int NT = DT * (DT + 1) / 2;
  constexpr int HEAD = 128;
  constexpr int TAIL = HEAD + NT * NB_TILE;
  constexpr int TC = (2 + 2 * DP + 127) / 128;
  constexpr int ELL_CHUNKS = 1 + 2 * NT + TC;
  static_assert(DP <= HEAD, "centre fits the head");
  static_assert(TAIL + TC * 128 <= FAST_REGION, "ellipsoid block fits a region");
  static_assert(KA * NB_HT1 * NB_TILE <= FAST_REGION, "layer-1 chunk fits");
  constexpr int NA_D = KA * NB_HT1 * NB_TILE;
  constexpr int NB1_D = (KT1 - KA) * NB_HT1 * NB_TILE;
  constexpr int NC_D = FAST_B_DOUBLES;
  extern __shared__ __attribute__((aligned(16))) double lds[];
  auto reg = [&](int i) __attribute__((always_inline)) {
    return lds + (i & 1) * FAST_REGION;
  };

  const int lane = threadIdx.x & 63;
  const int wave = __builtin_amdgcn_readfirstlane(threadIdx.x >> 6);
  const int lg = lane >> 4;
  const bool m_sample = a.sample != 0;
  const double* blob = a.blob;
  const int n_dim = (int)nb_hdr(blob, NB_H_NDIM);
  const int K = (int)nb_hdr(blob, NB_H_K);
  const bool use_cube = nb_hdr(blob, NB_H_USECUBE) != 0;
  const int ks1 = (n_dim + 1 + 3) >> 2;
  const long long net_stride = nb_hdr(blob, NB_H_NET_STRIDE);
  unsigned long long cnt_ell = 0, cnt_mlp = 0;
  long long sup = blockIdx.x;

  struct Pass {
    const double* nb;
    const double* shift;
    int E, b;
    long long base;
    int n_valid;
  };
  int* pp = (int*)(lds + 2 * FAST_REGION);
  long long n_super;
  if constexpr (BATCH) {
    if (wave == 0) {
      int run = 0;
      for (int g0 = 0; g0 < a.n_groups; g0 += 64) {
        const int g = g0 + lane;
        int v = g < a.n_groups ? (a.totals[g] + 127) >> 7 : 0;
#pragma unroll
        for (int d = 1; d < 64; d <<= 1) {
          const int u = __shfl_up(v, d);
          if (lane >= d) v += u;
        }
        if (g < a.n_groups) pp[g + 1] = run + v;
        run += __shfl(v, 63);
      }
      if (lane == 0) pp[0] = 0;
    }
    __syncthreads();
    n_super = pp[a.n_groups];
    if (sup >= n_super) return;
  } else {
    n_super = (a.n + 16 * NW * T - 1) / (16 * NW * T);
  }
  auto pass_of = [&](long long P) __attribute__((always_inline)) {
    Pass ps;
    if constexpr (BATCH) {
      const long long Pc = P < n_super ? P : n_super - 1;
      int lo = 0, hi = a.n_groups;
      while (hi - lo > 1) {
        const int mid = (lo + hi) >> 1;
        if (pp[mid] <= (int)Pc) lo = mid; else hi = mid;
      }
      const int g = __builtin_amdgcn_readfirstlane(lo);
      const FastGroup gd = a.groups[g];
      ps.nb = gd.nb;
      ps.shift = a.recentre != 0 ? gd.shift : nullptr;
      ps.E = gd.E;
      ps.b = gd.b;
      const int s0 = ((int)Pc - __builtin_amdgcn_readfirstlane(pp[g])) << 7;
      ps.base = (long long)g * a.n_pad + s0;
      const int left = a.totals[g] - s0;
      ps.n_valid = P < n_super ? (left < 128 ? left : 128) : 0;
    } else {
      ps.nb = blob + nb_hdr(blob, NB_H_OFF_NEURAL) +
              a.m * nb_hdr(blob, NB_H_NEURAL_STRIDE);
      ps.shift = (a.recentre != 0 && nb_hdr(blob, NB_H_OFF_SHIFT) != 0)
                     ? blob + nb_hdr(blob, NB_H_OFF_SHIFT) : nullptr;
      ps.E = (int)nb_hdr(blob, NB_H_E);
      ps.b = 0;
      ps.base = 0;
      ps.n_valid = 0;
    }
    return ps;
  };
  Pass cur_p = pass_of(sup);

  const double* dma_src = nullptr;
  double* dma_dst = nullptr;
  int dma_c = 0, dma_n = 0;
  bool dma_ell = false;
  auto dma_begin = [&](const double* src, double* dst, int n_doubles)
      __attribute__((always_inline)) {
    dma_src = src; dma_dst = dst; dma_c = wave; dma_n = n_doubles >> 7;
    dma_ell = false;
  };
  auto dma_begin_ell = [&](const double* nb_blk, double* dst)
      __attribute__((always_inline)) {
    dma_src = nb_blk; dma_dst = dst; dma_c = wave;
    dma_n = ELL_CHUNKS;
    dma_ell = true;
  };
  auto dma_one = [&]() __attribute__((always_inline)) {
    int s_off, d_off;
    if (!dma_ell) {
      s_off = d_off = dma_c * 128;
    } else if (dma_c < 1) {
      s_off = 2 + 2 * DP;
      d_off = 0;
    } else if (dma_c < 1 + 2 * NT) {
      const int p = (dma_c - 1) >> 1, half = (dma_c - 1) & 1;
      int ht = 0;
      while ((ht + 1) * (ht + 2) / 2 <= p) ++ht;
      const int kt = p - ht * (ht + 1) / 2;
      s_off = 2 + 3 * DP + (kt * DT + ht) * NB_TILE + half * 128;
      d_off = HEAD + p * NB_TILE + half * 128;
    } else {
      const int i = dma_c - 1 - 2 * NT;
      s_off = nb_ell_block_size(DT) + i * 128;
      d_off = TAIL + i * 128;
    }
    __builtin_amdgcn_global_load_lds(
        (nbf_gptr)(dma_src + s_off + 2 * lane),
        (nbf_lptr)(dma_dst + d_off), 16, 0, 0);
    dma_c += NW;
  };
  auto dma_tick = [&]() __attribute__((always_inline)) {
    if (dma_c < dma_n) dma_one();
  };
  auto dma_flush = [&]() __attribute__((always_inline)) {
    while (dma_c < dma_n) dma_one();
  };

  int q = 0;
  dma_begin_ell(cur_p.nb, reg(0));
  dma_flush();
  long long pt[T];
  bool valid[T];
  double2 xraw[T][2 * DT];
  auto row_of = [&](long long p) __attribute__((always_inline)) {
    return p < a.n ? (a.idx != nullptr ? a.idx[p] : p) : 0ll;
  };
  auto row_in = [&](const Pass& ps, int t) __attribute__((always_inline)) {
    const int slot = (wave * T + t) * 16 + (lane & 15);
    return (long long)a.dense[ps.base + (slot < ps.n_valid ? slot : 0)];
  };
  long long nrow[T];
#pragma unroll
  for (int t = 0; t < T; ++t) {
    pt[t] = ((sup * NW + wave) * T + t) * 16 + (lane & 15);
    valid[t] = pt[t] < a.n;
    if constexpr (BATCH) nrow[t] = row_in(cur_p, t);
    else nrow[t] = row_of(pt[t]);
  }
  load_points_raw<DT, T>(a.x, nrow, n_dim, lane, xraw);

  for (; sup < n_super; sup += gridDim.x) {
    const double* nb_m = cur_p.nb;
    const double* shift = cur_p.shift;
    const int E = cur_p.E;
    const double* nets = nb_m + nb_ell_block_size(DT) + 2 + 2 * DP;
    const Pass next_p = pass_of(sup + gridDim.x);
    int lgp = lg;
    asm volatile("" : "+v"(lgp));
    long long crow[T];
    dma_begin(nets, reg(q ^ 1), NA_D);
    dma_flush();
    asm volatile("s_waitcnt vmcnt(%0)" ::"n"((NA_D / 128 + NW - 1) / NW)
                 : "memory");
    __syncthreads();
    const double* blk = reg(q);
    const double thr = blk[TAIL];

    bool in_cube[T], acc_outer[T], want[T];
    double xin[T][4 * DT];
#pragma unroll
    for (int t = 0; t < T; ++t) {
      pt[t] = ((sup * NW + wave) * T + t) * 16 + (lane & 15);
      in_cube[t] = true;
      if constexpr (BATCH) {
        valid[t] = (wave * T + t) * 16 + (lane & 15) < cur_p.n_valid;
        crow[t] = nrow[t];
        nrow[t] = row_in(next_p, t);
      } else {
        valid[t] = pt[t] < a.n;
        nrow[t] = row_of((((sup + gridDim.x) * NW + wave) * T + t) * 16 +
                         (lane & 15));
      }
    }
    points_from_raw<DT, T>(xraw, valid, n_dim, lgp, xin);
    if (shift != nullptr) {
#pragma unroll
      for (int ks = 0; ks < 4 * DT; ++ks) {
        const double sv = shift[4 * ks + lgp];
        const bool on = shift[DP + 4 * ks + lgp] != 0.0;
#pragma unroll
        for (int t = 0; t < T; ++t) {
          const double v = xin[t][ks] + sv;
          xin[t][ks] = on ? v - floor(v) : xin[t][ks];
        }
      }
    }
    if (m_sample) {
      bool cbad[T];
#pragma unroll
      for (int t = 0; t < T; ++t) cbad[t] = false;
#pragma unroll
      for (int ks = 0; ks < 4 * DT; ++ks) {
        const int f = 8 * (ks >> 1) + 2 * lgp + (ks & 1);
        const bool boxed = use_cube && f < n_dim;
#pragma unroll
        for (int t = 0; t < T; ++t)
          cbad[t] |= boxed && !(xin[t][ks] >= 0.0 && xin[t][ks] < 1.0);
      }
#pragma unroll
      for (int t = 0; t < T; ++t) {
        in_cube[t] = !point_any(cbad[t], lane);
        acc_outer[t] = in_cube[t];
        want[t] = valid[t] && acc_outer[t];
      }
    } else {
#pragma unroll
      for (int t = 0; t < T; ++t) { acc_outer[t] = false; want[t] = valid[t]; }
    }

    double y[T][4 * DT], r2[T];
    bool box_bad[T], inside_e[T], need[T];
    ell_eval_centre<DT, T>(blk, blk + HEAD, n_dim, xin, lane, lgp, y, r2);
#pragma unroll
    for (int t = 0; t < T; ++t) box_bad[t] = false;
    bool wave_mlp = false;
#pragma unroll
    for (int t = 0; t < T; ++t) {
      inside_e[t] = !box_bad[t] && r2[t] < 1.0;
      need[t] = m_sample ? (want[t] && inside_e[t]) : valid[t];
      cnt_ell += __popcll(__ballot(want[t] && lg == 0));
      cnt_mlp += (unsigned long long)E * __popcll(__ballot(need[t] && lg == 0));
      wave_mlp |= need[t];
    }
    wave_mlp = __any(wave_mlp);

    double tin[T][KS1];
    {
      const double* r_mean = blk + TAIL + 2;
      const double* r_isc = r_mean + DP;
#pragma unroll
      for (int ks = 0; ks < KS1; ++ks) {
        const int f = 4 * ks + lgp;
        if (ks < 4 * DT) {
          const double mv = r_mean[f], sv = r_isc[f];
          const double pad = (f == n_dim) ? 1.0 : 0.0;
#pragma unroll
          for (int t = 0; t < T; ++t) {
            const double v = (y[t][ks] - mv) * sv;
            tin[t][ks] = (f < n_dim) ? v : pad;
          }
        } else {
#pragma unroll
          for (int t = 0; t < T; ++t) tin[t][ks] = (f == n_dim) ? 1.0 : 0.0;
        }
      }
    }
    asm volatile("s_waitcnt vmcnt(0)" ::: "memory");
    __syncthreads();
#pragma unroll
    for (int t = 0; t < T; ++t) asm volatile("" : "+v"(nrow[t]));

    double total[T];
#pragma unroll
    for (int t = 0; t < T; ++t) total[t] = 0.0;
    int cur = q ^ 1;

    auto stage_end = [&]() __attribute__((always_inline)) {
      dma_flush();
      asm volatile("s_waitcnt vmcnt(0)" ::: "memory");
      __syncthreads();
      cur ^= 1;
    };
    auto network = [&](int e, auto last_c) __attribute__((always_inline)) {
      constexpr bool LAST = decltype(last_c)::value;
      const double* w_e = nets + e * net_stride;
      double h1[T][4 * NB_HT1];
      if constexpr (TWO) {
        dma_begin(w_e + NA_D, reg(cur ^ 1), NB1_D);
        if (wave_mlp)
          fl_chunk<T, KS1, NB_HT1, 0, 4 * KA, 2>(reg(cur), ks1, tin, lane, h1,
                                                dma_tick);
        stage_end();
        dma_begin(w_e + NA_D + NB1_D, reg(cur ^ 1), NC_D);
        if (wave_mlp) {
          fl_chunk<T, KS1, NB_HT1, 4 * KA, KS1, 1>(reg(cur), ks1, tin, lane,
                                                  h1, dma_tick);
          fl_pad<T, NB_HT1, 25, 0>(h1, lane);
        }
        stage_end();
      } else {
        dma_begin(w_e + NA_D, reg(cur ^ 1), NC_D);
        if (wave_mlp) {
          fl_chunk<T, KS1, NB_HT1, 0, KS1, 1>(reg(cur), ks1, tin, lane, h1,
                                             dma_tick);
          fl_pad<T, NB_HT1, 25, 0>(h1, lane);
        }
        stage_end();
      }
      if constexpr (LAST) {
        load_points_raw<DT, T>(a.x, nrow, n_dim, lane, xraw);
        dma_begin_ell(next_p.nb, reg(cur ^ 1));
      } else {
        dma_begin(nets + (e + 1) * net_stride, reg(cur ^ 1), NA_D);
      }
      if (wave_mlp) {
        const double* w2 = reg(cur);
        const double* w3 = w2 + NB_HT1 * NB_HT2 * NB_TILE;
        const double* w4 = w3 + NB_HT2 * NB_HT3 * NB_TILE;
        double h2[T][4 * NB_HT2], h3[T][4 * NB_HT3], o[T][4];
        double a2[FlFirst<8, NB_HT2>::NA], a3[FlFirst<8, NB_HT3>::NA],
            a4[FlFirst<8, 1>::NA];
        fl_read_first<8, NB_HT2>(w2, lane, a2);
        fl_layer_from<T, 8, 26, 0, NB_HT2, true, 2, 1, 0>(
            w2, 26, h1, lane, h2, a2,
            [&]() __attribute__((always_inline)) {
              fl_read_first<8, NB_HT3>(w3, lane, a3);
            },
            dma_tick);
        fl_pad<T, NB_HT2, 12, 2>(h2, lane);
        fl_layer_from<T, 8, 13, 0, NB_HT3, true, 2, 2, 0>(
            w3, 13, h2, lane, h3, a3,
            [&]() __attribute__((always_inline)) {
              fl_read_first<8, 1>(w4, lane, a4);
            },
            dma_tick);
        fl_pad<T, NB_HT3, 5, 0>(h3, lane);
        fl_layer_from<T, 8, 6, 0, 1, true, 2, 5, 0>(
            w4, 6, h3, lane, o, a4, []() __attribute__((always_inline)) {},
            dma_tick);
#pragma unroll
        for (int t = 0; t < T; ++t) total[t] += o[t][0];
      }
      stage_end();
    };
    for (int e = 0; e + 1 < E; ++e) network(e, std::false_type{});
    network(E - 1, std::true_type{});
    q = cur;

#pragma unroll
    for (int t = 0; t < T; ++t) {
      const double score = __shfl(total[t], lane & 15) / (double)E;
      if constexpr (BATCH) {
        if (valid[t] && lg == 0 && score > thr) {
          a.st[crow[t]] = a.out_mode == 2 ? (unsigned char)3 : (unsigned char)2;
          if (a.out_mode == 1) atomicMin(&a.first[crow[t]], cur_p.b);
        }
      } else if (m_sample) {
        bool ok = inside_e[t];
        if (need[t]) ok = inside_e[t] && (score > thr);
        const unsigned char flags =
            (acc_outer[t] ? 1 : 0) | ((acc_outer[t] && ok) ? 2 : 0);
        if (valid[t] && lg == 0) a.out_u8[pt[t]] = flags;
      } else if (valid[t] && lg == 0) {
        a.out_f64[2 * pt[t]] = r2[t];
        a.out_f64[2 * pt[t] + 1] = score;
      }
    }
    cur_p = next_p;
  }
  if (a.counters != nullptr && lane == 0) {
    atomicAdd(&a.counters[1], cnt_ell);
    atomicAdd(&a.counters[2], cnt_mlp);
  }
}

template <int DT, int KT1, bool BATCH>
int launch_fast_impl(const FastArgs& a, hipStream_t stream) {
  const size_t lds = (size_t)2 * FAST_REGION * sizeof(double) +
                     (BATCH ? (FAST_MAX_GROUPS + 1) * sizeof(int) : 0);
  static bool configured = false;
  if (!configured) {
    const hipError_t e = hipFuncSetAttribute(
        (const void*)nb_eval_fast_kernel<DT, KT1, BATCH>,
        hipFuncAttributeMaxDynamicSharedMemorySize, (int)lds);
    if (e != hipSuccess) {
      nb_set_error("hipFuncSetAttribute(%zu bytes LDS) failed: %s", lds,
                   hipGetErrorString(e));
      return NB_ERR_HIP;
    }
    configured = true;
  }
  const long long n_super = (a.n + 127) / 128;
  long long blocks = n_super < 256 ? n_super : 256;
  hipLaunchKernelGGL((nb_eval_fast_kernel<DT, KT1, BATCH>),
                     dim3((unsigned)blocks), dim3(512), lds, stream, a);
  return NB_OK;
}

template <int DT, int KT1>
int launch_fast(const FastArgs& a, hipStream_t stream) {
  return a.groups != nullptr ? launch_fast_impl<DT, KT1, true>(a, stream)
                             : launch_fast_impl<DT, KT1, false>(a, stream);
}

}

unsigned long long* nb_eval_counters();

bool nb_eval_fast_eligible(int n_dim, int K, int M, int E, bool sample) {
  if (n_dim > 128 || M < 1 || E < 1) return false;
  return !sample || (K <= 1 && M == 1);
}

static int dispatch_fast(const FastArgs& a, int n_dim, hipStream_t stream) {
  const int dt = (n_dim + 15) / 16, kt1 = (n_dim + 1 + 15) / 16;
  int rc = NB_ERR_UNSUPPORTED;
  switch (4 * dt + (kt1 - dt)) {
    case 4: rc = launch_fast<1, 1>(a, stream); break;
    case 5: rc = launch_fast<1, 2>(a, stream); break;
    case 8: rc = launch_fast<2, 2>(a, stream); break;
    case 9: rc = launch_fast<2, 3>(a, stream); break;
    case 12: rc = launch_fast<3, 3>(a, stream); break;
    case 13: rc = launch_fast<3, 4>(a, stream); break;
    case 16: rc = launch_fast<4, 4>(a, stream); break;
    case 17: rc = launch_fast<4, 5>(a, stream); break;
    case 20: rc = launch_fast<5, 5>(a, stream); break;
    case 21: rc = launch_fast<5, 6>(a, stream); break;
    case 24: rc = launch_fast<6, 6>(a, stream); break;
    case 25: rc = launch_fast<6, 7>(a, stream); break;
    case 28: rc = launch_fast<7, 7>(a, stream); break;
    case 29: rc = launch_fast<7, 8>(a, stream); break;
    case 32: rc = launch_fast<8, 8>(a, stream); break;
    case 33: rc = launch_fast<8, 9>(a, stream); break;
    default:
      nb_set_error("nb_launch_eval_fast: n_dim=%d not eligible", n_dim);
      return NB_ERR_UNSUPPORTED;
  }
  if (rc != NB_OK) return rc;
  NB_HIP_CHECK(hipGetLastError());
  return NB_OK;
}

int nb_launch_eval_fast(const double* blob_dev, int n_dim, bool sample, int m,
                        int recentre, const double* x, const long long* idx,
                        long long n,
                        unsigned char* out_u8, double* out_f64,
                        unsigned long long seed, unsigned long long offset,
                        hipStream_t stream) {
  if (n <= 0) return NB_OK;
  FastArgs a = {};
  a.blob = blob_dev; a.sample = sample ? 1 : 0; a.x = (const nb_gd*)x; a.n = n;
  a.idx = idx; a.m = m; a.recentre = recentre;
  a.out_u8 = out_u8; a.out_f64 = out_f64; a.seed = seed; a.offset = offset;
  a.counters = nb_eval_counters();
  return dispatch_fast(a, n_dim, stream);
}

int nb_launch_eval_fast_batch(const double* blob0_dev, int n_dim, int recentre,
                              const double* x, const void* groups_dev,
                              int n_groups, const int* totals_dev,
                              const int* dense_dev, long long n_pad,
                              long long n_upper, int out_mode,
                              unsigned char* st, int* first,
                              hipStream_t stream) {
  if (n_upper <= 0 || n_groups <= 0) return NB_OK;
  if (n_groups > FAST_MAX_GROUPS) {
    nb_set_error("nb_launch_eval_fast_batch: %d groups (limit %d)", n_groups,
                 FAST_MAX_GROUPS);
    return NB_ERR_ARG;
  }
  FastArgs a = {};
  a.blob = blob0_dev; a.sample = 0; a.x = (const nb_gd*)x;
  a.n = n_upper + 128ll * n_groups;
  a.recentre = recentre;
  a.counters = nb_eval_counters();
  a.groups = (const FastGroup*)groups_dev; a.n_groups = n_groups;
  a.totals = totals_dev; a.dense = dense_dev; a.n_pad = n_pad;
  a.out_mode = out_mode; a.st = st; a.first = first;
  return dispatch_fast(a, n_dim, stream);
}
```

nautilus_amd/device.py:

```python

import ctypes as C
import math
import os
import time

import numpy as np
import torch
from scipy.linalg import solve_triangular

from . import _lib


try:
    _raw_stream = torch._C._cuda_getCurrentRawStream
    _cur_device = torch._C._cuda_getDevice
except AttributeError:
    _raw_stream = None


def _stream():
    if _raw_stream is None:
        return C.c_void_p(torch.cuda.current_stream().cuda_stream)
    return C.c_void_p(_raw_stream(_cur_device()))


def _itemsize(dtype):
    try:
        return dtype.itemsize
    except AttributeError:
        return torch.empty((), dtype=dtype).element_size()


def _ptr(t):
    return C.c_void_p(t.data_ptr())


def _f64(a):
    return np.ascontiguousarray(a, dtype=np.float64)


def _dp(a):
    return a.ctypes.data_as(_lib.c_double_p)


def as_device_points(x, n_dim=None):
    if isinstance(x, torch.Tensor):
        t = x.to(device='cuda', dtype=torch.float64)
    else:
        t = torch.from_numpy(_f64(x)).cuda()
    if t.dim() == 1:
        t = t.unsqueeze(0)
    t = t.contiguous()
    if n_dim is not None and t.shape[1] != n_dim:
        raise ValueError('points have %d columns, bound has n_dim=%d' %
                         (t.shape[1], n_dim))
    return t


def member(c=None, B=None, B_inv=None, idx_ell=None, free_dims=False):
    if c is None:
        return dict(n_ell=0, c=np.zeros(0), B=np.zeros((0, 0)),
                    B_inv=np.zeros((0, 0)), idx_ell=None, free_dims=free_dims)
    c = _f64(c)
    B = _f64(B)
    B_inv = _f64(np.linalg.inv(B) if B_inv is None else B_inv)
    B_inv = np.tril(B_inv)
    return dict(n_ell=len(c), c=c, B=np.tril(B), B_inv=B_inv,
                idx_ell=None if idx_ell is None else
                np.ascontiguousarray(idx_ell, dtype=np.int32),
                free_dims=free_dims)


class DeviceBound:

    def __init__(self, n_dim, members=(), log_v_all=None, unit_cube=False,
                 neural=(), shift=None):
        lib = _lib.load()
        self.n_dim = int(n_dim)
        self.n_members = len(members)
        self.n_neural = len(neural)
        keep = []

        def fill_member(md, src):
            md.n_ell = src['n_ell']
            md.free_dims = 1 if src.get('free_dims') else 0
            if src['idx_ell'] is not None:
                keep.append(src['idx_ell'])
                md.idx_ell = src['idx_ell'].ctypes.data_as(_lib.c_int32_p)
            else:
                md.idx_ell = None
            for key in ('c', 'B', 'B_inv'):
                arr = _f64(src[key])
                keep.append(arr)
                setattr(md, key, _dp(arr))

        m_arr = (_lib.MemberDesc * max(1, self.n_members))()
        for md, src in zip(m_arr, members):
            fill_member(md, src)
        n_arr = (_lib.NeuralDesc * max(1, self.n_neural))()
        self.n_networks = 0
        self.thresholds = [float(src.get('score_predict_min', 0.0)) - 1e-9
                           for src in neural]
        self.dense_need = None
        for nd, src in zip(n_arr, neural):
            fill_member(nd.ellipsoid, src['ellipsoid'])
            nd.score_predict_min = float(src.get('score_predict_min', 0.0))
            nd.radius2 = float(np.linalg.norm(src['ellipsoid']['B'], 2)**2 *
                               (1.0 + 1e-9))
            mlp = src.get('mlp')
            if mlp is None:
                nd.mlp = None
                continue
            e = len(mlp['nets'])
            self.n_networks = e
            md = _lib.MlpDesc()
            md.n_networks = e
            mean, scale = _f64(mlp['mean']), _f64(mlp['scale'])
            keep += [mean, scale]
            md.mean, md.scale = _dp(mean), _dp(scale)
            cp = (_lib.c_double_p * (4 * e))()
            ip = (_lib.c_double_p * (4 * e))()
            from .emulator import pad_network
            for i, (coefs, intercepts) in enumerate(mlp['nets']):
                coefs, intercepts = pad_network(coefs, intercepts, self.n_dim)
                for k in range(4):
                    w, b = _f64(coefs[k]), _f64(intercepts[k])
                    keep += [w, b]
                    cp[4 * i + k], ip[4 * i + k] = _dp(w), _dp(b)
            md.coefs, md.intercepts = cp, ip
            keep += [md, cp, ip]
            nd.mlp = C.pointer(md)

        desc = _lib.BoundDesc()
        desc.n_dim = self.n_dim
        desc.n_members = self.n_members
        desc.members = m_arr
        lv = _f64(np.zeros(self.n_members) if log_v_all is None
                  else log_v_all)
        desc.log_v_all = _dp(lv)
        desc.unit_cube = 1 if unit_cube else 0
        desc.n_neural = self.n_neural
        desc.neural = n_arr
        desc.n_periodic = 0
        if shift is not None and len(shift[0]) > 0:
            per = np.ascontiguousarray(shift[0], dtype=np.int32)
            cen = _f64(shift[1])
            keep += [per, cen]
            desc.n_periodic = len(per)
            desc.periodic = per.ctypes.data_as(_lib.c_int32_p)
            desc.centers = _dp(cen)
        handle = C.c_void_p()
        _lib.check(lib.nb_bound_create(C.byref(desc), C.byref(handle)))
        self._h = handle
        self._lib = lib
        del keep

    def __del__(self):
        h = getattr(self, '_h', None)
        if h:
            self._lib.nb_bound_destroy(h)
            self._h = None

    @property
    def nbytes(self):
        return self._lib.nb_bound_nbytes(self._h)

    def contains(self, x):
        x = as_device_points(x, self.n_dim)
        return (self._self_list().eval(x, GEOM_ANY)[0] & GS_INSIDE) != 0

    def _self_list(self):
        lst = self.__dict__.get('_list')
        if lst is None:
            lst = self._list = DeviceBoundList([self])
        return lst

    def contains_stream(self, x):
        x = as_device_points(x, self.n_dim)
        mask = torch.empty(x.shape[0], dtype=torch.uint8, device='cuda')
        _lib.check(self._lib.nb_ellipsoid_contains_stream(
            self._h, _ptr(x), x.shape[0], _ptr(mask), _stream()))
        return mask.bool()

    def transform(self, x):
        x = as_device_points(x, self.n_dim)
        y = torch.empty_like(x)
        _lib.check(self._lib.nb_ellipsoid_transform(
            self._h, _ptr(x), x.shape[0], _ptr(y), _stream()))
        return y

    def member_count(self, x):
        x = as_device_points(x, self.n_dim)
        cnt = torch.empty(x.shape[0], dtype=torch.uint8, device='cuda')
        _lib.check(self._lib.nb_member_count(self._h, _ptr(x), x.shape[0],
                                             _ptr(cnt), _stream()))
        return cnt

    def neural_score(self, x):
        x = as_device_points(x, self.n_dim)
        out = torch.empty((x.shape[0], 2), dtype=torch.float64, device='cuda')
        _lib.check(self._lib.nb_neural_score(self._h, _ptr(x), x.shape[0],
                                             _ptr(out), _stream()))
        return out[:, 0], out[:, 1]

    def propose(self, seed, offset, n, reuse=False):
        x = _buffer('propose', (n, self.n_dim), torch.float64, reuse)
        _lib.check(self._lib.nb_propose(self._h, seed, offset, n, _ptr(x),
                                        _stream()))
        return x

    def accept(self, seed, offset, x, reuse=False):
        fused_ok = (self.n_neural == 1 and self.n_members <= 1 and
                    self.n_networks >= 1)
        if fused_ok and self.dense_need is not None and self.dense_need > 0.5:
            flags = _buffer('accept', (x.shape[0],), torch.uint8, reuse)
            _lib.check(self._lib.nb_accept(self._h, seed, offset, _ptr(x),
                                           x.shape[0], _ptr(flags),
                                           _stream()))
            DISPATCHES['nb_eval_fast_kernel'] += 1
            return flags
        n = x.shape[0]
        flags = _buffer('accept', (n,), torch.uint8, reuse)
        need = self._lib.nb_accept_staged_work_bytes(self._h, n)
        work = _buffer('staged_work', (need,), torch.uint8, True)
        off = C.c_int64(0)
        _lib.check(self._lib.nb_accept_staged(
            self._h, seed, offset, _ptr(x), n, _ptr(flags), _ptr(work), need,
            C.byref(off), _stream()))
        DISPATCHES['nb_cand_kernel'] += 1
        DISPATCHES['nb_eval_fast_kernel'] += 1 if self.n_networks else 0
        if fused_ok and self.dense_need is None:
            totals = work[off.value:off.value + 4 * self.n_neural].view(
                torch.int32)
            self.dense_need = float(totals.sum()) / max(1, n)
        return flags

    def sample_launch(self, seed, offset, n_draw, mask=2, reuse=False,
                      out_role='compact'):
        x = self.propose(seed, offset, n_draw, reuse)
        flags = self.accept(seed, offset, x, reuse)
        out, counts, _ = compact_rows(x, flags, mask, reuse=reuse,
                                      out_role=out_role)
        return out, counts


class DeviceBoundList:

    def __init__(self, bounds):
        lib = _lib.load()
        self.bounds = list(bounds)
        arr = (C.c_void_p * max(1, len(self.bounds)))(
            *[b._h for b in self.bounds])
        handle = C.c_void_p()
        _lib.check(lib.nb_boundlist_create(arr, len(self.bounds),
                                           C.byref(handle)))
        self._h = handle
        self._lib = lib
        self.n_dim = self.bounds[0].n_dim if self.bounds else None

    def __del__(self):
        h = getattr(self, '_h', None)
        if h:
            self._lib.nb_boundlist_destroy(h)
            self._h = None

    def eval(self, x, mode, reuse=False):
        n = x.shape[0]
        st = _buffer('list_status', (n,), torch.uint8, reuse)
        first = (_buffer('list_first', (n,), torch.int32, reuse)
                 if mode == GEOM_FIRST else None)
        if n == 0:
            return st, first
        if len(self.bounds) == 0:
            st.zero_()
            if first is not None:
                first.fill_(NO_BOUND)
            return st, first
        slab = n
        while slab > 4096 and self._lib.nb_list_eval_work_bytes(
                self._h, slab) > WORK_BYTES:
            slab = (slab + 1) // 2
        need = max(self._lib.nb_list_eval_work_bytes(self._h, slab),
                   self._lib.nb_list_eval_work_bytes(
                       self._h, n - (n - 1) // slab * slab))
        work = _buffer('staged_work', (need,), torch.uint8, True)
        for lo in range(0, n, slab):
            k = min(slab, n - lo)
            _lib.check(self._lib.nb_list_eval(
                self._h, mode, _ptr(x[lo:]), k, _ptr(st[lo:]),
                _ptr(first[lo:]) if first is not None else None, _ptr(work),
                need, _stream()))
            DISPATCHES['nb_cand_kernel'] += 1
            DISPATCHES['nb_eval_fast_kernel'] += 1
        return st, first

    def inside_flags(self, x, reuse=False):
        return self.eval(as_device_points(x, self.n_dim), GEOM_ANY, reuse)[0]

    def contains_any(self, x, as_flags=False):
        x = as_device_points(x, self.n_dim)
        st, _ = self.eval(x, GEOM_ANY)
        inside = (st & GS_INSIDE) != 0
        return inside.to(torch.uint8) if as_flags else inside

    def first_containing(self, x):
        x = as_device_points(x, self.n_dim)
        _, first = self.eval(x, GEOM_FIRST)
        return torch.where(first == NO_BOUND, torch.full_like(first, -1),
                           first)


GEOM_ANY, GEOM_FIRST, GEOM_SAMPLE = 0, 1, 2
NO_BOUND = 2**31 - 1
WORK_BYTES = 256 << 20
DISPATCHES = dict(nb_eval_fast_kernel=0, nb_cand_kernel=0)
GS_OUTER, GS_INSIDE = 1, 2


MAX_DIM = 128


def _work(n_doubles):
    return torch.empty(int(n_doubles), dtype=torch.float64, device='cuda')


def mvee_weights(x, n_max=100, n_batch=20):
    lib = _lib.load()
    x = as_device_points(x)
    n, d = x.shape
    u = torch.empty(n, dtype=torch.float64, device='cuda')
    work = _work(lib.nb_mvee_weights_work_doubles(n, d, n_batch))
    _lib.check(lib.nb_mvee_weights(_ptr(x), n, d, n_max, n_batch, _ptr(u),
                                   _ptr(work), _stream()))
    return u


def weighted_moments(x, w=None, scale=1.0):
    lib = _lib.load()
    x = as_device_points(x)
    n, d = x.shape
    out = torch.empty((d + 1, d + 1), dtype=torch.float64, device='cuda')
    work = _work(lib.nb_moments_work_doubles(n, d))
    _lib.check(lib.nb_weighted_moments(
        _ptr(x), _ptr(w) if w is not None else None, n, d, float(scale),
        _ptr(out), _ptr(work), _stream()))
    return out


def quadform_max(x, p):
    lib = _lib.load()
    x = as_device_points(x)
    n, d = x.shape
    p = torch.as_tensor(p, dtype=torch.float64).to('cuda').contiguous()
    out = torch.empty(1, dtype=torch.float64, device='cuda')
    work = _work(lib.nb_quadform_work_doubles())
    _lib.check(lib.nb_quadform_max(_ptr(x), n, d, _ptr(p), _ptr(out),
                                   _ptr(work), _stream()))
    return out


def whiten(x):
    lib = _lib.load()
    x = as_device_points(x)
    n, d = x.shape
    xw = torch.empty_like(x)
    stats = torch.empty(2 * d + d * d, dtype=torch.float64, device='cuda')
    work = _work(lib.nb_whiten_work_doubles(n, d))
    _lib.check(lib.nb_whiten(
        _ptr(x), n, d, _ptr(xw), _ptr(stats), _ptr(stats[d:]),
        _ptr(stats[2 * d:]), _ptr(work), _stream()))
    return xw, stats


def mvee_fit_batch(point_sets, n_max=100, n_batch=20):
    lib = _lib.load()
    xs, stats, us = [], [], []
    for pts in point_sets:
        xw, st = whiten(pts)
        xs.append(xw)
        stats.append(st)
        us.append(torch.empty(xw.shape[0], dtype=torch.float64,
                              device='cuda'))
    nb = len(xs)
    d = xs[0].shape[1]
    n_arr = (C.c_int64 * nb)(*[x.shape[0] for x in xs])
    work = _work(lib.nb_mvee_work_doubles(nb, max(n_arr), d, n_batch))
    _lib.check(lib.nb_mvee_khachiyan(
        nb, (C.c_void_p * nb)(*[x.data_ptr() for x in xs]), n_arr, d, n_max,
        n_batch, (C.c_void_p * nb)(*[u.data_ptr() for u in us]), _ptr(work),
        _stream()))
    moments = torch.stack([weighted_moments(x, u) for x, u in zip(xs, us)])
    moments = moments.cpu().numpy()
    stats = torch.stack(stats).cpu().numpy()
    p_all, c_all, cov_all = [], [], []
    for s in moments:
        su = s[d, d]
        c = s[d, :d] / su
        cov = s[:d, :d] / su - np.outer(c, c)
        cov = 0.5 * (cov + cov.T)
        v = np.empty((d + 1, d + 1))
        v[:d, :d] = s[:d, :d] / su
        v[d, :d] = v[:d, d] = c
        v[d, d] = 1.0
        p_all.append(np.linalg.inv(v))
        c_all.append(c)
        cov_all.append(cov)
    gmax = torch.cat([quadform_max(x, p) for x, p in zip(xs, p_all)])
    gmax = gmax.cpu().numpy()
    out = []
    for b in range(nb):
        mean, sd = stats[b, :d], stats[b, d:2 * d]
        w = stats[b, 2 * d:].reshape(d, d)
        back = sd[:, None] * solve_triangular(w, np.eye(d), lower=True)
        fwd = w / sd[None, :]
        scale = gmax[b] - 1.0
        c = mean + back @ c_all[b]
        a_inv = back @ cov_all[b] @ back.T * scale
        a = fwd.T @ np.linalg.inv(cov_all[b]) @ fwd / scale
        out.append((c, 0.5 * (a + a.T), 0.5 * (a_inv + a_inv.T)))
    return out


def standardize(x):
    lib = _lib.load()
    x = as_device_points(x)
    n, d = x.shape
    mean = torch.empty(d, dtype=torch.float64, device='cuda')
    scale = torch.empty(d, dtype=torch.float64, device='cuda')
    out = torch.empty_like(x)
    _lib.check(lib.nb_standardize(_ptr(x), n, d, _ptr(mean), _ptr(scale),
                                  _ptr(out), _stream()))
    return mean, scale, out


def prior_transform(u, kind, loc, scale):
    lib = _lib.load()
    u = as_device_points(u)
    n, d = u.shape
    out = torch.empty_like(u)
    kind = np.ascontiguousarray(kind, dtype=np.uint8)
    loc, scale = _f64(loc), _f64(scale)
    _lib.check(lib.nb_prior_transform(
        _ptr(u), n, d, kind.ctypes.data_as(C.c_void_p), _dp(loc), _dp(scale),
        _ptr(out), _stream()))
    return out



ROW_MAJOR, COLUMN_MAJOR = 0, 1


class PriorTable:

    def __init__(self, kind, loc, scale, shape0, shape1, key_column,
                 key_value):
        self._lib = lib = _lib.load()
        kind = np.ascontiguousarray(kind, dtype=np.uint8)
        arrays = [_f64(a) for a in (loc, scale, shape0, shape1)]
        key_column = np.ascontiguousarray(key_column, dtype=np.int32)
        key_value = _f64(key_value)
        self.n_dim, self.n_keys = len(kind), len(key_column)
        if any(len(a) != self.n_dim for a in arrays) or \
                len(key_value) != self.n_keys:
            raise ValueError('prior table arrays differ in length')
        h = C.c_void_p()
        _lib.check(lib.nb_prior_table_create(
            self.n_dim, kind.ctypes.data_as(C.c_void_p),
            *[_dp(a) for a in arrays], self.n_keys,
            key_column.ctypes.data_as(_lib.c_int32_p), _dp(key_value),
            C.byref(h)))
        self._h = h

    def __del__(self):
        h = getattr(self, '_h', None)
        if h:
            self._lib.nb_prior_table_destroy(h)
            self._h = None

    def transform(self, u, layout=ROW_MAJOR):
        u = as_device_points(u, self.n_dim)
        n = u.shape[0]
        shape = (n, self.n_dim) if layout == ROW_MAJOR else (self.n_keys, n)
        out = torch.empty(shape, dtype=torch.float64, device=u.device)
        _lib.check(self._lib.nb_prior_table_transform(
            self._h, _ptr(u), n, layout, _ptr(out), _stream()))
        return out




def gmm_fit(x, n_init=10, seed=0, tol=1e-3, reg_covar=1e-6, max_iter=100,
            init_labels=None):
    lib = _lib.load()
    x = as_device_points(x)
    n, d = x.shape
    stride = lib.nb_gmm_out_doubles(d)
    out = torch.zeros(n_init * stride, dtype=torch.float64, device='cuda')
    scratch = torch.empty(lib.nb_gmm_work_doubles(n, d, n_init),
                          dtype=torch.float64, device='cuda')
    lab = None
    if init_labels is not None:
        lab = torch.from_numpy(np.ascontiguousarray(
            init_labels, dtype=np.int32).reshape(n_init, n)).cuda()
    _lib.check(lib.nb_gmm_fit(
        _ptr(x), n, d, n_init, int(seed) & (2**64 - 1), float(tol),
        float(reg_covar), int(max_iter), _ptr(lab) if lab is not None else None,
        _ptr(out), _ptr(scratch), _stream()))
    rec = out.cpu().numpy().reshape(n_init, stride)
    per = lib.nb_gmm_scratch_doubles(n, d)
    off = lib.nb_gmm_logp_offset(d)
    fits = []
    for i, r in enumerate(rec):
        fits.append(dict(
            lower_bound=float(r[0]), n_iter=int(r[1]), converged=bool(r[2]),
            failed=bool(r[3]), weights=r[4:6].copy(),
            means=r[6:6 + 2 * d].reshape(2, d).copy(),
            covariances=r[6 + 2 * d:].reshape(2, d, d).copy(),
            logp=scratch[i * per + off:i * per + off + 2 * n].view(2, n)))
    return fits


def phase_shift_(x, periodic, centers, inverse=False):
    lib = _lib.load()
    if x.shape[0] == 0 or len(periodic) == 0:
        return x
    assert x.is_cuda and x.dtype == torch.float64 and x.is_contiguous()
    per = np.ascontiguousarray(periodic, dtype=np.int32)
    cen = _f64(centers)
    _lib.check(lib.nb_phase_shift(
        _ptr(x), x.shape[0], x.shape[1], len(per),
        per.ctypes.data_as(_lib.c_int32_p), _dp(cen), 1 if inverse else 0,
        _stream()))
    return x


_SCRATCH = {}


def _buffer(role, shape, dtype, reuse):
    if not reuse:
        return torch.empty(shape, dtype=dtype, device='cuda')
    n_bytes = math.prod(shape) * _itemsize(dtype)
    buf = _SCRATCH.get(role)
    if buf is None or buf.numel() < n_bytes:
        _SCRATCH[role] = buf = None
        buf = torch.empty(n_bytes + n_bytes // 4 + 512, dtype=torch.uint8,
                          device='cuda')
        _SCRATCH[role] = buf
    return buf[:n_bytes].view(dtype).view(shape)


def compact_rows(x, flags, mask=1, want_index=False, reuse=False, flip=0,
                 out_role='compact'):
    lib = _lib.load()
    n, d = x.shape
    out = _buffer(out_role, (n, d), torch.float64, reuse)
    counts = torch.empty(2, dtype=torch.int64, device='cuda')
    scratch = _buffer('compact_scratch',
                      (max(16, lib.nb_compact_scratch_bytes(n)),),
                      torch.uint8, reuse)
    src = (_buffer('compact_index', (n,), torch.int64, reuse)
           if want_index else None)
    _lib.check(lib.nb_compact_rows(
        _ptr(x), _ptr(flags), mask, flip, n, d, _ptr(out),
        _ptr(src) if src is not None else None, _ptr(counts), _ptr(scratch),
        _stream()))
    return out, counts, src


def shell_stats(log_l, threshold=-np.inf):
    lib = _lib.load()
    n = log_l.shape[0]
    out = torch.empty(4, dtype=torch.float64, device='cuda')
    scratch = torch.empty(max(16, lib.nb_shell_stats_scratch_bytes(n)),
                          dtype=torch.uint8, device='cuda')
    _lib.check(lib.nb_shell_stats(_ptr(log_l), n, float(threshold), _ptr(out),
                                  _ptr(scratch), _stream()))
    return out


class LivePool:

    def __init__(self, k, tensors=()):
        self._lib = _lib.load()
        self.k = int(k)
        self._host = np.array([-np.inf, 0.0, 0.0, 0.0])
        self._alloc(sum(int(t.shape[0]) for t in tensors) + 16)
        for t in tensors:
            self.add(t)
        if self.dirty:
            self.select()
        keep = self.bufs[self.cur][:int(self.counts[self.cur])].clone()
        thr = self.thr.clone()
        self._alloc(max(4 * self.k, 2 * int(keep.shape[0])) + (1 << 17))
        self.bufs[0][:keep.shape[0]] = keep
        self.counts[0] = keep.shape[0]
        self.thr.copy_(thr)

    def _alloc(self, capacity):
        self.cap = int(capacity)
        self.bufs = [torch.empty(self.cap, dtype=torch.float64, device='cuda')
                     for _ in range(2)]
        self.counts = torch.zeros(3, dtype=torch.int32, device='cuda')
        self.thr = torch.full((1,), -np.inf, dtype=torch.float64,
                              device='cuda')
        self.stats = torch.zeros(4, dtype=torch.float64, device='cuda')
        self.cur = 0
        self.dirty = False

    def add(self, log_l):
        if log_l.shape[0] == 0:
            return
        log_l = log_l.contiguous()
        _lib.check(self._lib.nb_live_append(
            _ptr(log_l), log_l.shape[0], _ptr(self.thr), _ptr(self.bufs[
                self.cur]), _ptr(self.counts[self.cur:]), self.cap,
            _ptr(self.counts[2:]), _stream()))
        self.dirty = True

    def select(self):
        if self.dirty:
            nxt = 1 - self.cur
            _lib.check(self._lib.nb_live_select(
                _ptr(self.bufs[self.cur]), _ptr(self.counts[self.cur:]),
                self.cap, self.k, _ptr(self.bufs[nxt]),
                _ptr(self.counts[nxt:]), _ptr(self.thr), _ptr(self.stats),
                _stream()))
            self.cur = nxt
            self.dirty = False
            self._host = torch.cat([self.stats[:3],
                                    self.counts[2:].double()]).cpu().numpy()
            if self._host[3] != 0:
                raise OverflowError('live pool capacity exceeded')
        return float(self._host[0]), int(self._host[1]), int(self._host[2])

    def select_with_stats(self, shells):
        if not self.dirty:
            return self.select(), self.shell_stats(shells)
        nxt = 1 - self.cur
        _lib.check(self._lib.nb_live_select(
            _ptr(self.bufs[self.cur]), _ptr(self.counts[self.cur:]),
            self.cap, self.k, _ptr(self.bufs[nxt]),
            _ptr(self.counts[nxt:]), _ptr(self.thr), _ptr(self.stats),
            _stream()))
        self.cur = nxt
        self.dirty = False
        out = torch.zeros((max(1, len(shells)), 4), dtype=torch.float64,
                          device='cuda')
        for row, ll in zip(out, shells):
            _lib.check(self._lib.nb_live_stats(
                _ptr(ll), ll.shape[0], _ptr(self.thr), _ptr(row), _stream()))
        host = torch.cat([self.stats[:3], self.counts[2:].double(),
                          out[:len(shells), :3].reshape(-1)]).cpu().numpy()
        self._host = host[:4]
        if self._host[3] != 0:
            raise OverflowError('live pool capacity exceeded')
        return ((float(host[0]), int(host[1]), int(host[2])),
                host[4:].reshape(len(shells), 3))

    def smallest_above(self):
        vals = self.bufs[self.cur][:int(self.counts[self.cur])]
        return float(vals[vals > self.thr].min())

    def shell_stats(self, shells):
        out = torch.zeros((max(1, len(shells)), 4), dtype=torch.float64,
                          device='cuda')
        for row, ll in zip(out, shells):
            _lib.check(self._lib.nb_live_stats(
                _ptr(ll), ll.shape[0], _ptr(self.thr), _ptr(row), _stream()))
        return out[:len(shells), :3].cpu().numpy()


def philox_uniform(seed, offset, block, tag, n):
    lib = _lib.load()
    u = torch.empty((n, 2), dtype=torch.float64, device='cuda')
    _lib.check(lib.nb_philox_uniform(seed, offset, block, tag, n, _ptr(u),
                                     _stream()))
    return u


def mfma_f64_peak(iters=20000):
    lib = _lib.load()
    out = C.c_double(0.0)
    _lib.check(lib.nb_mfma_f64_peak(iters, C.byref(out)))
    return out.value


class EvalCounters:

    def __init__(self):
        self._lib = _lib.load()
        self.buf = torch.zeros(4, dtype=torch.int64, device='cuda')

    def __enter__(self):
        self.buf.zero_()
        _lib.check(self._lib.nb_set_eval_counters(_ptr(self.buf)))
        return self

    def __exit__(self, *exc):
        torch.cuda.synchronize()
        _lib.check(self._lib.nb_set_eval_counters(None))

    def read(self):
        c = self.buf.cpu().numpy()
        return dict(outer_point_evals=int(c[0]), ellipsoid_point_evals=int(c[1]),
                    emulator_point_evals=int(c[2]))


class KernelTimer:

    active = None

    def __init__(self):
        self.events = {}
        self.folded = {}

    def __enter__(self):
        KernelTimer.active = self
        return self

    def __exit__(self, *exc):
        KernelTimer.active = None

    def _fold(self, name):
        pairs = self.events.pop(name, [])
        if pairs:
            pairs[-1][1].synchronize()
            acc = self.folded.setdefault(name, [0, 0.0])
            acc[0] += len(pairs)
            acc[1] += sum(a.elapsed_time(b) for a, b in pairs)

    def totals(self):
        torch.cuda.synchronize()
        for name in list(self.events):
            self._fold(name)
        return {name: dict(launches=acc[0], ms=acc[1])
                for name, acc in self.folded.items()}


def _timed(name):
    def deco(fn):
        def wrapper(*args, **kwargs):
            timer = KernelTimer.active
            if timer is None:
                return fn(*args, **kwargs)
            a = torch.cuda.Event(enable_timing=True)
            b = torch.cuda.Event(enable_timing=True)
            a.record()
            out = fn(*args, **kwargs)
            b.record()
            pairs = timer.events.setdefault(name, [])
            pairs.append((a, b))
            if len(pairs) >= 1024:
                timer._fold(name)
            return out
        wrapper.__name__ = fn.__name__
        wrapper.__doc__ = fn.__doc__
        return wrapper
    return deco


DeviceBound.contains = _timed('bound_eval')(DeviceBound.contains)
DeviceBound.accept = _timed('bound_eval')(DeviceBound.accept)
DeviceBound.neural_score = _timed('bound_eval')(DeviceBound.neural_score)
DeviceBound.propose = _timed('nb_draw_kernel')(DeviceBound.propose)
DeviceBound.contains_stream = _timed('nb_ell_stream_kernel')(
    DeviceBound.contains_stream)
DeviceBoundList.contains_any = _timed('bound_eval')(
    DeviceBoundList.contains_any)
DeviceBoundList.inside_flags = _timed('bound_eval')(
    DeviceBoundList.inside_flags)
DeviceBoundList.first_containing = _timed('bound_eval')(
    DeviceBoundList.first_containing)
compact_rows = _timed('nb_compact')(compact_rows)
shell_stats = _timed('nb_lse')(shell_stats)
```

Baseline: 2.548 million.

## Add fp32 neural-emulator screen with rigorous error bounds before fp64 evaluation

Adds a screening kernel that evaluates the neural acceptance networks in single precision using packed fp32 weight tiles. Per-layer constants derived from the weights bound the rounding error, so the kernel can decide most points outright and compacts only the undecided ones. Those go to the existing fp64 fast batch kernel. This aims to cut fp64 MLP cost on the accept path, at the price of an extra kernel, a compaction pass and more blob memory. A runtime check switches screening off when too large a share of points stays undecided.

Measured after the change: 2.539 million. About the same (-0.4%).

```diff
diff --git a/include/nautilus_hip.h b/include/nautilus_hip.h
--- a/include/nautilus_hip.h
+++ b/include/nautilus_hip.h
@@ -218,6 +218,18 @@
                          const double* x_dev, const int64_t* idx_dev,
                          int64_t n, double* out_dev, void* stream);
 
+int64_t nb_accept_screened_work_bytes(const nb_bound* bound, int64_t n);
+int nb_accept_screened(const nb_bound* bound, uint64_t seed, uint64_t offset,
+                       const double* x_dev, int64_t n, uint8_t* flags_dev,
+                       void* work_dev, int64_t work_bytes,
+                       int64_t* count_offset, void* stream);
+int nb_screen_score(const nb_bound* bound, const double* x_dev, int64_t n,
+                    double* out_dev, void* stream);
+int64_t nb_screen_net_floats(int32_t n_dim);
+int nb_screen_pack(int32_t n_dim, const double* const* coefs_host,
+                   const double* const* intercepts_host, float* tiles_host,
+                   double* consts_host);
+
 int64_t nb_gmm_out_doubles(int32_t n_dim);
 int64_t nb_gmm_scratch_doubles(int64_t n, int32_t n_dim);
 int64_t nb_gmm_work_doubles(int64_t n, int32_t n_dim, int32_t n_init);
diff --git a/nautilus_amd/_lib.py b/nautilus_amd/_lib.py
--- a/nautilus_amd/_lib.py
+++ b/nautilus_amd/_lib.py
@@ -176,6 +176,17 @@
     'nb_neural_score_rows': (C.c_int, [C.c_void_p, C.c_int32, C.c_int32,
                                        C.c_void_p, C.c_void_p, C.c_int64,
                                        C.c_void_p, C.c_void_p]),
+    'nb_accept_screened_work_bytes': (C.c_int64, [C.c_void_p, C.c_int64]),
+    'nb_accept_screened': (C.c_int, [C.c_void_p, C.c_uint64, C.c_uint64,
+                                     C.c_void_p, C.c_int64, C.c_void_p,
+                                     C.c_void_p, C.c_int64,
+                                     C.POINTER(C.c_int64), C.c_void_p]),
+    'nb_screen_score': (C.c_int, [C.c_void_p, C.c_void_p, C.c_int64,
+                                  C.c_void_p, C.c_void_p]),
+    'nb_screen_net_floats': (C.c_int64, [C.c_int32]),
+    'nb_screen_pack': (C.c_int, [C.c_int32, C.POINTER(c_double_p),
+                                 C.POINTER(c_double_p), C.c_void_p,
+                                 c_double_p]),
     'nb_gmm_out_doubles': (C.c_int64, [C.c_int32]),
     'nb_gmm_scratch_doubles': (C.c_int64, [C.c_int64, C.c_int32]),
     'nb_gmm_work_doubles': (C.c_int64, [C.c_int64, C.c_int32, C.c_int32]),
diff --git a/nautilus_amd/csrc/nb_api.hip b/nautilus_amd/csrc/nb_api.hip
--- a/nautilus_amd/csrc/nb_api.hip
+++ b/nautilus_amd/csrc/nb_api.hip
@@ -35,6 +35,11 @@
                               long long n_upper, int out_mode,
                               unsigned char* st, int* first,
                               hipStream_t stream);
+long long nb_screen_work_bytes(long long n);
+int nb_launch_screen(const double* blob_dev, int n_dim, bool sample,
+                     const double* x, long long n, unsigned char* out_u8,
+                     double* out_f64, int* work, int** dense_out,
+                     int** totals_out, hipStream_t stream);
 int nb_launch_eval(int dt, const double* const* blobs_dev, int nb, int mode,
                    const double* x, long long n, unsigned char* out_u8,
                    int* out_i32, double* out_f64, unsigned long long seed,
@@ -137,6 +142,7 @@
   bool single_full_ellipsoid = false;
   int64_t off_stream = 0;
   int64_t off_members = 0, off_neural = 0;
+  int64_t off_screen = 0;
 };
 
 static inline int64_t nb_hdr_host_off_members(const nb_bound* b) {
@@ -264,6 +270,61 @@
   put_weight(w4, 1, NB_H3, 0, intercepts[3][0]);
 }
 
+inline int screen_col(int u) { return 4 * (u & 3) + (u >> 2); }
+
+void put_weight32(float* tiles, int ht_n, int k, int h, double v) {
+  tiles[((size_t)(k >> 4) * ht_n + (h >> 4)) * NB_TILE + (k & 15) * 16 +
+        screen_col(h & 15)] = (float)v;
+}
+
+void screen_layer_consts(const double* w, const double* b, int K, int H,
+                         double* a_out, double* b_out) {
+  double fro2 = 0.0, n1 = 0.0, ninf = 0.0;
+  std::vector<double> col(H, 0.0);
+  for (int k = 0; k < K; ++k) {
+    double row = 0.0;
+    for (int h = 0; h < H; ++h) {
+      const double v = std::fabs(w[(size_t)k * H + h]);
+      fro2 += v * v;
+      row += v;
+      col[h] += v;
+    }
+    ninf = std::fmax(ninf, row);
+  }
+  for (int h = 0; h < H; ++h) n1 = std::fmax(n1, col[h]);
+  double bias2 = 0.0;
+  for (int h = 0; h < H; ++h) bias2 += b[h] * b[h];
+  const double up = 1.0 + 1e-9;
+  const int n = 4 * ((K + 1 + 3) / 4);
+  const double u = 5.9604644775390625e-8;
+  const double g = (n + 1) * u / (1.0 - (n + 1) * u) * up;
+  const double A = g * std::sqrt(fro2 + bias2) * up;
+  const double P = std::fmin(std::sqrt(fro2), std::sqrt(n1 * ninf)) * up;
+  *a_out = A;
+  *b_out = (P + 2.0 * A) * up;
+}
+
+void fill_net32(float* net, double* consts, int n_dim, int kt1,
+                const double* const* coefs, const double* const* intercepts) {
+  float* w1 = net;
+  float* w2 = w1 + (size_t)kt1 * NB_HT1 * NB_TILE;
+  float* w3 = w2 + (size_t)NB_HT1 * NB_HT2 * NB_TILE;
+  float* w4 = w3 + (size_t)NB_HT2 * NB_HT3 * NB_TILE;
+  float* const w[4] = {w1, w2, w3, w4};
+  const int K[4] = {n_dim, NB_H1, NB_H2, NB_H3};
+  const int H[4] = {NB_H1, NB_H2, NB_H3, 1};
+  const int HT[4] = {NB_HT1, NB_HT2, NB_HT3, 1};
+  for (int l = 0; l < 4; ++l) {
+    for (int k = 0; k < K[l]; ++k)
+      for (int h = 0; h < H[l]; ++h)
+        put_weight32(w[l], HT[l], k, h, coefs[l][(size_t)k * H[l] + h]);
+    for (int h = 0; h < H[l]; ++h)
+      put_weight32(w[l], HT[l], K[l], h, intercepts[l][h]);
+    screen_layer_consts(coefs[l], intercepts[l], K[l], H[l], &consts[l],
+                        &consts[4 + l]);
+  }
+}
+
 inline hipStream_t as_stream(void* s) { return (hipStream_t)s; }
 
 }
@@ -328,6 +389,9 @@
   }
   const int64_t off_shift = off;
   if (d->n_periodic > 0) off += 2 * dp;
+  const bool screen = (M == 1 && E >= 1);
+  const int64_t off_screen = off;
+  if (screen) off += (int64_t)E * (net_stride / 2) + 8 * (int64_t)E;
   const int64_t total = off;
 
   std::vector<double> buf((size_t)total, 0.0);
@@ -351,6 +415,7 @@
   put_i64(buf, NB_H_TOTAL, total);
   put_i64(buf, NB_H_OFF_STREAM, single_full ? off_stream : 0);
   put_i64(buf, NB_H_OFF_SHIFT, d->n_periodic > 0 ? off_shift : 0);
+  put_i64(buf, NB_H_OFF_SCREEN, screen ? off_screen : 0);
   for (int i = 0; i < d->n_periodic; ++i) {
     const int f = d->periodic[i];
     if (f < 0 || f >= n_dim) {
@@ -472,6 +537,12 @@
       for (int e = 0; e < E; ++e)
         fill_net(scale + dp + (size_t)e * net_stride, n_dim, kt1,
                  nd.mlp->coefs + 4 * e, nd.mlp->intercepts + 4 * e);
+      if (screen)
+        for (int e = 0; e < E; ++e)
+          fill_net32((float*)&buf[off_screen + (size_t)e * (net_stride / 2)],
+                     &buf[off_screen + (size_t)E * (net_stride / 2) + 8 * e],
+                     n_dim, kt1, nd.mlp->coefs + 4 * e,
+                     nd.mlp->intercepts + 4 * e);
     }
   }
 
@@ -483,6 +554,7 @@
   b->off_members = off_members;
   b->off_neural = off_neural;
   b->off_shift = nb_hdr(buf.data(), NB_H_OFF_SHIFT);
+  b->off_screen = nb_hdr(buf.data(), NB_H_OFF_SCREEN);
   b->neural_stride = nb_hdr(buf.data(), NB_H_NEURAL_STRIDE);
   constexpr size_t SLACK = 512;
   hipError_t e = hipMalloc((void**)&b->blob_dev,
@@ -844,6 +916,72 @@
 #endif
   return nb_launch_eval(b->dt, b->self_list_dev, 1, 2, x, n, flags, nullptr,
                         nullptr, seed, offset, as_stream(stream));
+}
+
+static bool nb_screen_eligible(const nb_bound* b) {
+  return b->off_screen != 0 &&
+         nb_eval_fast_eligible(b->n_dim, b->K, b->M, b->E, true);
+}
+
+int64_t nb_screen_net_floats(int32_t n_dim) {
+  return (int64_t)nb_net_tiles((n_dim + 1 + 15) / 16) * NB_TILE;
+}
+
+int nb_screen_pack(int32_t n_dim, const double* const* coefs,
+                   const double* const* intercepts, float* tiles,
+                   double* consts) {
+  if (n_dim < 1 || n_dim > 16 * NB_MAX_DT || coefs == nullptr ||
+      intercepts == nullptr || tiles == nullptr || consts == nullptr) {
+    nb_set_error("nb_screen_pack: bad argument");
+    return NB_ERR_ARG;
+  }
+  std::memset(tiles, 0, (size_t)nb_screen_net_floats(n_dim) * sizeof(float));
+  fill_net32(tiles, consts, n_dim, (n_dim + 1 + 15) / 16, coefs, intercepts);
+  return NB_OK;
+}
+
+int64_t nb_accept_screened_work_bytes(const nb_bound* b, int64_t n) {
+  (void)b;
+  return nb_screen_work_bytes(n);
+}
+
+int nb_accept_screened(const nb_bound* b, uint64_t seed, uint64_t offset,
+                       const double* x, int64_t n, uint8_t* flags, void* work,
+                       int64_t work_bytes, int64_t* count_offset,
+                       void* stream) {
+  (void)seed; (void)offset;
+  if (!nb_screen_eligible(b)) {
+    nb_set_error("nb_accept_screened: needs one neural bound with networks "
+                 "and at most one outer member");
+    return NB_ERR_UNSUPPORTED;
+  }
+  if (n <= 0) return NB_OK;
+  if (n > 0x7fffffffll || work_bytes < nb_screen_work_bytes(n)) {
+    nb_set_error("nb_accept_screened: n = %lld, work space of %lld bytes, "
+                 "need %lld", (long long)n, (long long)work_bytes,
+                 (long long)nb_screen_work_bytes(n));
+    return NB_ERR_ARG;
+  }
+  int *dense = nullptr, *totals = nullptr;
+  int rc = nb_launch_screen(b->blob_dev, b->n_dim, true, x, n, flags, nullptr,
+                            (int*)work, &dense, &totals, as_stream(stream));
+  if (rc != NB_OK) return rc;
+  if (count_offset != nullptr)
+    *count_offset = (int64_t)((char*)totals - (char*)work);
+  return nb_launch_eval_fast_batch(b->blob_dev, b->n_dim, 0, x, b->groups_dev,
+                                   1, totals, dense, n, n, 2, flags, nullptr,
+                                   as_stream(stream));
+}
+
+int nb_screen_score(const nb_bound* b, const double* x, int64_t n, double* out,
+                    void* stream) {
+  if (!nb_screen_eligible(b)) {
+    nb_set_error("nb_screen_score: needs one neural bound with networks and "
+                 "at most one outer member");
+    return NB_ERR_UNSUPPORTED;
+  }
+  return nb_launch_screen(b->blob_dev, b->n_dim, false, x, n, nullptr, out,
+                          nullptr, nullptr, nullptr, as_stream(stream));
 }
 
 int64_t nb_compact_scratch_bytes(int64_t n) {
diff --git a/nautilus_amd/csrc/nb_common.h b/nautilus_amd/csrc/nb_common.h
--- a/nautilus_amd/csrc/nb_common.h
+++ b/nautilus_amd/csrc/nb_common.h
@@ -31,7 +31,8 @@
   NB_H_NDIM = 0, NB_H_DT, NB_H_K, NB_H_USECUBE, NB_H_M, NB_H_E, NB_H_OFF_CDF,
   NB_H_OFF_ULO, NB_H_OFF_UHI, NB_H_OFF_MEMBERS, NB_H_ELL_STRIDE,
   NB_H_OFF_NEURAL, NB_H_NEURAL_STRIDE, NB_H_OFF_DRAW, NB_H_DRAW_STRIDE,
-  NB_H_NET_STRIDE, NB_H_KT1, NB_H_TOTAL, NB_H_OFF_STREAM, NB_H_OFF_SHIFT
+  NB_H_NET_STRIDE, NB_H_KT1, NB_H_TOTAL, NB_H_OFF_STREAM, NB_H_OFF_SHIFT,
+  NB_H_OFF_SCREEN
 };
 
 __host__ __device__ inline int64_t nb_hdr(const double* blob, int i) {
diff --git a/nautilus_amd/csrc/nb_eval_fast.hip b/nautilus_amd/csrc/nb_eval_fast.hip
--- a/nautilus_amd/csrc/nb_eval_fast.hip
+++ b/nautilus_amd/csrc/nb_eval_fast.hip
@@ -2,7 +2,7 @@
 
 #include <type_traits>
 
-#include "nb_mlp.h"
+#include "nb_fast.h"
 
 namespace {
 
@@ -33,122 +33,6 @@
 
 constexpr int FAST_B_DOUBLES =
     (NB_HT1 * NB_HT2 + NB_HT2 * NB_HT3 + NB_HT3) * NB_TILE;
-
-typedef const void __attribute__((address_space(1))) * nbf_gptr;
-typedef void __attribute__((address_space(3))) * nbf_lptr;
-
-template <int DT, int T>
-__device__ __forceinline__ void ell_eval_centre(
-    const double* c, const double* tiles, int n_dim,
-    const double (&xin)[T][4 * DT], int lane, int lg, double (&y)[T][4 * DT],
-    double (&r2)[T]) {
-  double d[T][4 * DT];
-#pragma unroll
-  for (int ks = 0; ks < 4 * DT; ++ks) {
-    const double cv = c[4 * ks + lg];
-#pragma unroll
-    for (int t = 0; t < T; ++t) d[t][ks] = xin[t][ks] - cv;
-  }
-  double part[T];
-#pragma unroll
-  for (int t = 0; t < T; ++t) part[t] = 0.0;
-  const int live = n_dim - 16 * (DT - 1);
-  const bool small = DT > 1 && live >= 1 && live <= 4;
-  const int lane4 = (lane >> 4) * 16 + (lane & 3);
-#pragma unroll
-  for (int ht = 0; ht < DT; ++ht) {
-    if (ht == DT - 1 && small) {
-      double r4[T];
-#pragma unroll
-      for (int t = 0; t < T; ++t) r4[t] = 0.0;
-#pragma unroll
-      for (int ks = 0; ks < 4 * (ht + 1) - 2; ++ks) {
-        const int kt = ks >> 2, s = ks & 3;
-        const double a =
-            tiles[(ht * (ht + 1) / 2 + kt) * NB_TILE + s * 64 + lane4];
-#pragma unroll
-        for (int t = 0; t < T; ++t) r4[t] = NB_MFMA4(a, d[t][ks], r4[t]);
-      }
-#pragma unroll
-      for (int t = 0; t < T; ++t) {
-        y[t][4 * ht] = r4[t];
-        y[t][4 * ht + 1] = y[t][4 * ht + 2] = y[t][4 * ht + 3] = 0.0;
-        part[t] += r4[t] * r4[t];
-      }
-    } else if (16 * ht < n_dim) {
-      nb_d4 acc[T];
-#pragma unroll
-      for (int t = 0; t < T; ++t) acc[t] = nb_d4{0.0, 0.0, 0.0, 0.0};
-#pragma unroll
-      for (int ks = 0; ks < 4 * (ht + 1); ++ks) {
-        const int kt = ks >> 2, s = ks & 3;
-        const double a =
-            tiles[(ht * (ht + 1) / 2 + kt) * NB_TILE + s * 64 + lane];
-#pragma unroll
-        for (int t = 0; t < T; ++t) acc[t] = MFMA(a, d[t][ks], acc[t]);
-      }
-#pragma unroll
-      for (int t = 0; t < T; ++t)
-#pragma unroll
-        for (int r = 0; r < 4; ++r) {
-          y[t][4 * ht + r] = acc[t][r];
-          part[t] += acc[t][r] * acc[t][r];
-        }
-    } else {
-#pragma unroll
-      for (int t = 0; t < T; ++t)
-#pragma unroll
-        for (int r = 0; r < 4; ++r) y[t][4 * ht + r] = 0.0;
-    }
-  }
-#pragma unroll
-  for (int t = 0; t < T; ++t) r2[t] = lane_group_sum(part[t]);
-}
-
-template <int DT, int T>
-__device__ __forceinline__ void load_points_raw(
-    const nb_gd* __restrict__ x, const long long (&row_of)[T], int n_dim,
-    int lane, double2 (&raw)[T][2 * DT]) {
-  int lg = lane >> 4;
-  asm volatile("" : "+v"(lg));
-  asm volatile("" : "+s"(x));
-  if ((n_dim & 1) == 0) {
-#pragma unroll
-    for (int t = 0; t < T; ++t) {
-      const nb_gd* row = x + row_of[t] * n_dim;
-#pragma unroll
-      for (int j = 0; j < 2 * DT; ++j) {
-        const int f = 8 * j + 2 * lg;
-        raw[t][j] = *(const NB_G double2*)(row + (f < n_dim ? f : n_dim - 2));
-      }
-    }
-  } else {
-#pragma unroll
-    for (int t = 0; t < T; ++t) {
-      const nb_gd* row = x + row_of[t] * n_dim;
-#pragma unroll
-      for (int j = 0; j < 2 * DT; ++j) {
-        const int f = 8 * j + 2 * lg;
-        raw[t][j].x = row[f < n_dim ? f : n_dim - 1];
-        raw[t][j].y = row[f + 1 < n_dim ? f + 1 : n_dim - 1];
-      }
-    }
-  }
-}
-
-template <int DT, int T>
-__device__ __forceinline__ void points_from_raw(
-    const double2 (&raw)[T][2 * DT], const bool (&valid)[T], int n_dim,
-    int lg, double (&xin)[T][4 * DT]) {
-#pragma unroll
-  for (int t = 0; t < T; ++t)
-#pragma unroll
-    for (int j = 0; j < 2 * DT; ++j) {
-      const int f = 8 * j + 2 * lg;
-      xin[t][2 * j] = (valid[t] && f < n_dim) ? raw[t][j].x : 0.0;
-      xin[t][2 * j + 1] = (valid[t] && f + 1 < n_dim) ? raw[t][j].y : 0.0;
-    }
-}
 
 constexpr int FAST_REGION = 38 * NB_TILE;
 
diff --git a/nautilus_amd/csrc/nb_fast.h b/nautilus_amd/csrc/nb_fast.h
--- /dev/null
+++ b/nautilus_amd/csrc/nb_fast.h
@@ -0,0 +1,124 @@
+#pragma once
+#include "nb_common.h"
+
+#include "nb_mlp.h"
+
+namespace {
+
+typedef const void __attribute__((address_space(1))) * nbf_gptr;
+typedef void __attribute__((address_space(3))) * nbf_lptr;
+
+template <int DT, int T>
+__device__ __forceinline__ void ell_eval_centre(
+    const double* c, const double* tiles, int n_dim,
+    const double (&xin)[T][4 * DT], int lane, int lg, double (&y)[T][4 * DT],
+    double (&r2)[T]) {
+  double d[T][4 * DT];
+#pragma unroll
+  for (int ks = 0; ks < 4 * DT; ++ks) {
+    const double cv = c[4 * ks + lg];
+#pragma unroll
+    for (int t = 0; t < T; ++t) d[t][ks] = xin[t][ks] - cv;
+  }
+  double part[T];
+#pragma unroll
+  for (int t = 0; t < T; ++t) part[t] = 0.0;
+  const int live = n_dim - 16 * (DT - 1);
+  const bool small = DT > 1 && live >= 1 && live <= 4;
+  const int lane4 = (lane >> 4) * 16 + (lane & 3);
+#pragma unroll
+  for (int ht = 0; ht < DT; ++ht) {
+    if (ht == DT - 1 && small) {
+      double r4[T];
+#pragma unroll
+      for (int t = 0; t < T; ++t) r4[t] = 0.0;
+#pragma unroll
+      for (int ks = 0; ks < 4 * (ht + 1) - 2; ++ks) {
+        const int kt = ks >> 2, s = ks & 3;
+        const double a =
+            tiles[(ht * (ht + 1) / 2 + kt) * NB_TILE + s * 64 + lane4];
+#pragma unroll
+        for (int t = 0; t < T; ++t) r4[t] = NB_MFMA4(a, d[t][ks], r4[t]);
+      }
+#pragma unroll
+      for (int t = 0; t < T; ++t) {
+        y[t][4 * ht] = r4[t];
+        y[t][4 * ht + 1] = y[t][4 * ht + 2] = y[t][4 * ht + 3] = 0.0;
+        part[t] += r4[t] * r4[t];
+      }
+    } else if (16 * ht < n_dim) {
+      nb_d4 acc[T];
+#pragma unroll
+      for (int t = 0; t < T; ++t) acc[t] = nb_d4{0.0, 0.0, 0.0, 0.0};
+#pragma unroll
+      for (int ks = 0; ks < 4 * (ht + 1); ++ks) {
+        const int kt = ks >> 2, s = ks & 3;
+        const double a =
+            tiles[(ht * (ht + 1) / 2 + kt) * NB_TILE + s * 64 + lane];
+#pragma unroll
+        for (int t = 0; t < T; ++t) acc[t] = MFMA(a, d[t][ks], acc[t]);
+      }
+#pragma unroll
+      for (int t = 0; t < T; ++t)
+#pragma unroll
+        for (int r = 0; r < 4; ++r) {
+          y[t][4 * ht + r] = acc[t][r];
+          part[t] += acc[t][r] * acc[t][r];
+        }
+    } else {
+#pragma unroll
+      for (int t = 0; t < T; ++t)
+#pragma unroll
+        for (int r = 0; r < 4; ++r) y[t][4 * ht + r] = 0.0;
+    }
+  }
+#pragma unroll
+  for (int t = 0; t < T; ++t) r2[t] = lane_group_sum(part[t]);
+}
+
+template <int DT, int T>
+__device__ __forceinline__ void load_points_raw(
+    const nb_gd* __restrict__ x, const long long (&row_of)[T], int n_dim,
+    int lane, double2 (&raw)[T][2 * DT]) {
+  int lg = lane >> 4;
+  asm volatile("" : "+v"(lg));
+  asm volatile("" : "+s"(x));
+  if ((n_dim & 1) == 0) {
+#pragma unroll
+    for (int t = 0; t < T; ++t) {
+      const nb_gd* row = x + row_of[t] * n_dim;
+#pragma unroll
+      for (int j = 0; j < 2 * DT; ++j) {
+        const int f = 8 * j + 2 * lg;
+        raw[t][j] = *(const NB_G double2*)(row + (f < n_dim ? f : n_dim - 2));
+      }
+    }
+  } else {
+#pragma unroll
+    for (int t = 0; t < T; ++t) {
+      const nb_gd* row = x + row_of[t] * n_dim;
+#pragma unroll
+      for (int j = 0; j < 2 * DT; ++j) {
+        const int f = 8 * j + 2 * lg;
+        raw[t][j].x = row[f < n_dim ? f : n_dim - 1];
+        raw[t][j].y = row[f + 1 < n_dim ? f + 1 : n_dim - 1];
+      }
+    }
+  }
+}
+
+template <int DT, int T>
+__device__ __forceinline__ void points_from_raw(
+    const double2 (&raw)[T][2 * DT], const bool (&valid)[T], int n_dim,
+    int lg, double (&xin)[T][4 * DT]) {
+#pragma unroll
+  for (int t = 0; t < T; ++t)
+#pragma unroll
+    for (int j = 0; j < 2 * DT; ++j) {
+      const int f = 8 * j + 2 * lg;
+      xin[t][2 * j] = (valid[t] && f < n_dim) ? raw[t][j].x : 0.0;
+      xin[t][2 * j + 1] = (valid[t] && f + 1 < n_dim) ? raw[t][j].y : 0.0;
+    }
+}
+
+}
diff --git a/nautilus_amd/csrc/nb_mlp32.h b/nautilus_amd/csrc/nb_mlp32.h
--- /dev/null
+++ b/nautilus_amd/csrc/nb_mlp32.h
@@ -0,0 +1,92 @@
+#pragma once
+#include "nb_common.h"
+
+typedef float nb_f4 __attribute__((ext_vector_type(4)));
+#define MFMA32(a, b, c) \
+  __builtin_amdgcn_mfma_f32_16x16x4f32((a), (b), (c), 0, 0, 0)
+#define NB_TILE32 256
+
+namespace {
+
+template <int HT>
+__device__ __forceinline__ void sl_read_a(const float* w, int ks, int lane,
+                                          float (&a)[HT]) {
+  const float* wk = w + (ks >> 2) * HT * NB_TILE32 + (ks & 3) * 64;
+#pragma unroll
+  for (int h = 0; h < HT; ++h) a[h] = wk[h * NB_TILE32 + lane];
+}
+
+template <int KSMAX, int NGUARD, int HT, bool RELU_IN, int TICK_P, int PD,
+          int NIN, class Next, class Tick>
+__device__ __forceinline__ void sl_layer(const float* w, int ks_n,
+                                         const float (&in)[NIN], int lane,
+                                         float (&out)[4 * HT],
+                                         const float (&a0)[HT], Next&& next,
+                                         Tick&& tick) {
+  constexpr int KS_U = KSMAX - NGUARD;
+  static_assert(KS_U >= 1 && KS_U >= PD && PD >= 1, "prefetch distance");
+  static_assert(NIN >= KSMAX, "one B operand per k-step");
+  constexpr int R = PD + 1;
+  nb_f4 acc[HT];
+#pragma unroll
+  for (int h = 0; h < HT; ++h) acc[h] = nb_f4{0.f, 0.f, 0.f, 0.f};
+  auto step = [&](int ks, const float (&a)[HT]) __attribute__((always_inline)) {
+    const float b = RELU_IN ? fmaxf(in[ks], 0.f) : in[ks];
+#pragma unroll
+    for (int h = 0; h < HT; ++h) acc[h] = MFMA32(a[h], b, acc[h]);
+  };
+  auto arrived = [&](const float (&a)[HT]) __attribute__((always_inline)) {
+#pragma unroll
+    for (int i = 0; i < HT; ++i) asm volatile("" ::"v"(a[i]));
+  };
+  float a[R][HT];
+#pragma unroll
+  for (int i = 0; i < HT; ++i) a[0][i] = a0[i];
+#pragma unroll
+  for (int i = 1; i < PD; ++i) sl_read_a<HT>(w, i, lane, a[i]);
+  __builtin_amdgcn_sched_barrier(0);
+#pragma unroll
+  for (int ks = 0; ks < KS_U; ++ks) {
+    arrived(a[ks % R]);
+    __builtin_amdgcn_sched_barrier(0);
+    if (ks + PD < KS_U)
+      sl_read_a<HT>(w, ks + PD, lane, a[(ks + PD) % R]);
+    else if (ks + PD == KS_U) next();
+    if (ks % TICK_P == 0) tick();
+    __builtin_amdgcn_sched_barrier(0);
+    step(ks, a[ks % R]);
+    __builtin_amdgcn_sched_barrier(0);
+  }
+#pragma unroll
+  for (int ks = KS_U; ks < KSMAX; ++ks) {
+    if (ks < ks_n) {
+      float ag[HT];
+      sl_read_a<HT>(w, ks, lane, ag);
+      step(ks, ag);
+    }
+  }
+#pragma unroll
+  for (int h = 0; h < HT; ++h)
+#pragma unroll
+    for (int r = 0; r < 4; ++r) out[4 * h + r] = acc[h][r];
+}
+
+template <int ONE_KS, int ONE_LG, int NOUT>
+__device__ __forceinline__ void sl_one(float (&out)[NOUT], int lane) {
+  if ((lane >> 4) == ONE_LG) out[ONE_KS] = 1.f;
+}
+
+template <int N>
+__device__ __forceinline__ float sl_sumsq(const float (&h)[N], bool relu) {
+  float s = 0.f;
+#pragma unroll
+  for (int i = 0; i < N; ++i) {
+    const float v = relu ? fmaxf(h[i], 0.f) : h[i];
+    s = fmaf(v, v, s);
+  }
+  s += __shfl_xor(s, 16);
+  s += __shfl_xor(s, 32);
+  return s;
+}
+
+}
diff --git a/nautilus_amd/csrc/nb_screen.hip b/nautilus_amd/csrc/nb_screen.hip
--- /dev/null
+++ b/nautilus_amd/csrc/nb_screen.hip
@@ -0,0 +1,426 @@
+#include "nb_common.h"
+
+#include "nb_fast.h"
+#include "nb_mlp32.h"
+
+namespace {
+
+constexpr int SCR_REGION = 38 * NB_TILE;
+constexpr int SCR_BLOCKS = 256;
+constexpr int SCR_NW = 8;
+constexpr int SCR_SEGS = SCR_BLOCKS * SCR_NW;
+constexpr int SCR_C_D =
+    (NB_HT1 * NB_HT2 + NB_HT2 * NB_HT3 + NB_HT3) * NB_TILE32 / 2;
+
+struct ScreenArgs {
+  const double* blob;
+  int sample;
+  const nb_gd* x;
+  long long n;
+  unsigned char* out_u8;
+  double* out_f64;
+  int* seg;
+  int* seg_count;
+  long long seg_cap;
+  unsigned long long* counters;
+};
+
+template <int DT, int KT1>
+__global__ void __launch_bounds__(512) nb_screen_kernel(ScreenArgs a) {
+  constexpr int T = 1, NW = SCR_NW, DP = 16 * DT;
+  constexpr int KS1 = 4 * KT1;
+  constexpr int NT = DT * (DT + 1) / 2;
+  constexpr int HEAD = 128;
+  constexpr int TAIL = HEAD + NT * NB_TILE;
+  constexpr int TC = (2 + 2 * DP + 127) / 128;
+  constexpr int ELL_CHUNKS = 1 + 2 * NT + TC;
+  static_assert(DP <= HEAD, "centre fits the head");
+  static_assert(TAIL + TC * 128 <= SCR_REGION, "ellipsoid block fits a region");
+  constexpr int NA_D = KT1 * NB_HT1 * NB_TILE32 / 2;
+  constexpr int NC_D = SCR_C_D;
+  static_assert(NA_D <= SCR_REGION && NC_D <= SCR_REGION, "a stage fits");
+  extern __shared__ __attribute__((aligned(16))) double lds[];
+  auto reg = [&](int i) __attribute__((always_inline)) {
+    return lds + (i & 1) * SCR_REGION;
+  };
+
+  const int lane = threadIdx.x & 63;
+  const int wave = __builtin_amdgcn_readfirstlane(threadIdx.x >> 6);
+  const int lg = lane >> 4;
+  const bool m_sample = a.sample != 0;
+  const double* blob = a.blob;
+  const int n_dim = (int)nb_hdr(blob, NB_H_NDIM);
+  const bool use_cube = nb_hdr(blob, NB_H_USECUBE) != 0;
+  const int ks1 = (n_dim + 1 + 3) >> 2;
+  const int E = (int)nb_hdr(blob, NB_H_E);
+  const long long net_stride = nb_hdr(blob, NB_H_NET_STRIDE) / 2;
+  const double* nb_m = blob + nb_hdr(blob, NB_H_OFF_NEURAL);
+  const double* nets = blob + nb_hdr(blob, NB_H_OFF_SCREEN);
+  const double* consts = nets + E * net_stride;
+  unsigned long long cnt_ell = 0, cnt_scr = 0;
+  long long sup = blockIdx.x;
+  const long long n_super = (a.n + 16 * NW * T - 1) / (16 * NW * T);
+  int* my_seg = a.seg + (long long)(blockIdx.x * NW + wave) * a.seg_cap;
+  int n_und = 0;
+
+  const double* dma_src = nullptr;
+  double* dma_dst = nullptr;
+  int dma_c = 0, dma_n = 0;
+  bool dma_ell = false;
+  auto dma_begin = [&](const double* src, double* dst, int n_doubles)
+      __attribute__((always_inline)) {
+    dma_src = src; dma_dst = dst; dma_c = wave; dma_n = n_doubles >> 7;
+    dma_ell = false;
+  };
+  auto dma_begin_ell = [&](const double* nb_blk, double* dst)
+      __attribute__((always_inline)) {
+    dma_src = nb_blk; dma_dst = dst; dma_c = wave;
+    dma_n = ELL_CHUNKS;
+    dma_ell = true;
+  };
+  auto dma_one = [&]() __attribute__((always_inline)) {
+    int s_off, d_off;
+    if (!dma_ell) {
+      s_off = d_off = dma_c * 128;
+    } else if (dma_c < 1) {
+      s_off = 2 + 2 * DP;
+      d_off = 0;
+    } else if (dma_c < 1 + 2 * NT) {
+      const int p = (dma_c - 1) >> 1, half = (dma_c - 1) & 1;
+      int ht = 0;
+      while ((ht + 1) * (ht + 2) / 2 <= p) ++ht;
+      const int kt = p - ht * (ht + 1) / 2;
+      s_off = 2 + 3 * DP + (kt * DT + ht) * NB_TILE + half * 128;
+      d_off = HEAD + p * NB_TILE + half * 128;
+    } else {
+      const int i = dma_c - 1 - 2 * NT;
+      s_off = nb_ell_block_size(DT) + i * 128;
+      d_off = TAIL + i * 128;
+    }
+    __builtin_amdgcn_global_load_lds(
+        (nbf_gptr)(dma_src + s_off + 2 * lane),
+        (nbf_lptr)(dma_dst + d_off), 16, 0, 0);
+    dma_c += NW;
+  };
+  auto dma_tick = [&]() __attribute__((always_inline)) {
+    if (dma_c < dma_n) dma_one();
+  };
+  auto dma_flush = [&]() __attribute__((always_inline)) {
+    while (dma_c < dma_n) dma_one();
+  };
+
+  int q = 0;
+  dma_begin_ell(nb_m, reg(0));
+  dma_flush();
+  long long pt[T];
+  bool valid[T];
+  double2 xraw[T][2 * DT];
+  auto row_of = [&](long long p) __attribute__((always_inline)) {
+    return p < a.n ? p : 0ll;
+  };
+  long long nrow[T];
+#pragma unroll
+  for (int t = 0; t < T; ++t) {
+    pt[t] = ((sup * NW + wave) * T + t) * 16 + (lane & 15);
+    valid[t] = pt[t] < a.n;
+    nrow[t] = row_of(pt[t]);
+  }
+  load_points_raw<DT, T>(a.x, nrow, n_dim, lane, xraw);
+
+  for (; sup < n_super; sup += gridDim.x) {
+    int lgp = lg;
+    asm volatile("" : "+v"(lgp));
+    dma_begin(nets, reg(q ^ 1), NA_D);
+    dma_flush();
+    asm volatile("s_waitcnt vmcnt(%0)" ::"n"((NA_D / 128 + NW - 1) / NW)
+                 : "memory");
+    __syncthreads();
+    const double* blk = reg(q);
+    const double thr = blk[TAIL];
+
+    bool in_cube[T], acc_outer[T], want[T];
+    double xin[T][4 * DT];
+#pragma unroll
+    for (int t = 0; t < T; ++t) {
+      pt[t] = ((sup * NW + wave) * T + t) * 16 + (lane & 15);
+      in_cube[t] = true;
+      valid[t] = pt[t] < a.n;
+      nrow[t] = row_of((((sup + gridDim.x) * NW + wave) * T + t) * 16 +
+                       (lane & 15));
+    }
+    points_from_raw<DT, T>(xraw, valid, n_dim, lgp, xin);
+    if (m_sample) {
+      bool cbad[T];
+#pragma unroll
+      for (int t = 0; t < T; ++t) cbad[t] = false;
+#pragma unroll
+      for (int ks = 0; ks < 4 * DT; ++ks) {
+        const int f = 8 * (ks >> 1) + 2 * lgp + (ks & 1);
+        const bool boxed = use_cube && f < n_dim;
+#pragma unroll
+        for (int t = 0; t < T; ++t)
+          cbad[t] |= boxed && !(xin[t][ks] >= 0.0 && xin[t][ks] < 1.0);
+      }
+#pragma unroll
+      for (int t = 0; t < T; ++t) {
+        in_cube[t] = !point_any(cbad[t], lane);
+        acc_outer[t] = in_cube[t];
+        want[t] = valid[t] && acc_outer[t];
+      }
+    } else {
+#pragma unroll
+      for (int t = 0; t < T; ++t) { acc_outer[t] = false; want[t] = valid[t]; }
+    }
+
+    double y[T][4 * DT], r2[T];
+    bool inside_e[T], need[T];
+    ell_eval_centre<DT, T>(blk, blk + HEAD, n_dim, xin, lane, lgp, y, r2);
+    bool wave_mlp = false;
+#pragma unroll
+    for (int t = 0; t < T; ++t) {
+      inside_e[t] = r2[t] < 1.0;
+      need[t] = m_sample ? (want[t] && inside_e[t]) : valid[t];
+      cnt_ell += __popcll(__ballot(want[t] && lg == 0));
+      cnt_scr += (unsigned long long)E * __popcll(__ballot(need[t] && lg == 0));
+      wave_mlp |= need[t];
+    }
+    wave_mlp = __any(wave_mlp);
+
+    float tin[KS1];
+    {
+      const double* r_mean = blk + TAIL + 2;
+      const double* r_isc = r_mean + DP;
+#pragma unroll
+      for (int ks = 0; ks < KS1; ++ks) {
+        const int f = 4 * ks + lgp;
+        if (ks < 4 * DT) {
+          const double mv = r_mean[f], sv = r_isc[f];
+          const float pad = (f == n_dim) ? 1.f : 0.f;
+          const double v = (y[0][ks] - mv) * sv;
+          tin[ks] = (f < n_dim) ? (float)v : pad;
+        } else {
+          tin[ks] = (f == n_dim) ? 1.f : 0.f;
+        }
+      }
+    }
+    constexpr float UP = 1.f + 1.52587890625e-5f;
+    const double na0 = (double)(sqrtf(sl_sumsq(tin, false)) * UP);
+    asm volatile("s_waitcnt vmcnt(0)" ::: "memory");
+    __syncthreads();
+#pragma unroll
+    for (int t = 0; t < T; ++t) asm volatile("" : "+v"(nrow[t]));
+
+    double total = 0.0, delta = 0.0;
+    int cur = q ^ 1;
+
+    auto stage_end = [&]() __attribute__((always_inline)) {
+      dma_flush();
+      asm volatile("s_waitcnt vmcnt(0)" ::: "memory");
+      __syncthreads();
+      cur ^= 1;
+    };
+    auto network = [&](int e, auto last_c) __attribute__((always_inline)) {
+      constexpr bool LAST = decltype(last_c)::value;
+      const double* w_e = nets + e * net_stride;
+      const double* ce = consts + 8 * e;
+      float h1[4 * NB_HT1];
+      dma_begin(w_e + NA_D, reg(cur ^ 1), NC_D);
+      if (wave_mlp) {
+        const float* w1 = (const float*)reg(cur);
+        float a1[NB_HT1];
+        sl_read_a<NB_HT1>(w1, 0, lane, a1);
+        sl_layer<KS1, 3, NB_HT1, false, 1, 1>(
+            w1, ks1, tin, lane, h1, a1, []() __attribute__((always_inline)) {},
+            dma_tick);
+        sl_one<25, 0>(h1, lane);
+      }
+      stage_end();
+      if constexpr (LAST) {
+        load_points_raw<DT, T>(a.x, nrow, n_dim, lane, xraw);
+        dma_begin_ell(nb_m, reg(cur ^ 1));
+      } else {
+        dma_begin(nets + (e + 1) * net_stride, reg(cur ^ 1), NA_D);
+      }
+      if (wave_mlp) {
+        const float* w2 = (const float*)reg(cur);
+        const float* w3 = w2 + NB_HT1 * NB_HT2 * NB_TILE32;
+        const float* w4 = w3 + NB_HT2 * NB_HT3 * NB_TILE32;
+        float h2[4 * NB_HT2], h3[4 * NB_HT3], o[4];
+        float a2[NB_HT2], a3[NB_HT3], a4[1];
+        sl_read_a<NB_HT2>(w2, 0, lane, a2);
+        const float s1 = sl_sumsq(h1, true);
+        sl_layer<26, 0, NB_HT2, true, 2, 2>(
+            w2, 26, h1, lane, h2, a2,
+            [&]() __attribute__((always_inline)) {
+              sl_read_a<NB_HT3>(w3, 0, lane, a3);
+            },
+            dma_tick);
+        sl_one<12, 2>(h2, lane);
+        const float s2 = sl_sumsq(h2, true);
+        sl_layer<13, 0, NB_HT3, true, 2, 3>(
+            w3, 13, h2, lane, h3, a3,
+            [&]() __attribute__((always_inline)) {
+              sl_read_a<1>(w4, 0, lane, a4);
+            },
+            dma_tick);
+        sl_one<5, 0>(h3, lane);
+        const float s3 = sl_sumsq(h3, true);
+        sl_layer<6, 0, 1, true, 2, 5>(
+            w4, 6, h3, lane, o, a4, []() __attribute__((always_inline)) {},
+            dma_tick);
+        total += (double)o[0];
+        constexpr double TINY = 1e-30;
+        double err = 5.9604644775390625e-8 * na0 + TINY;
+        err = ce[0] * na0 + ce[4] * err + TINY;
+        err = ce[1] * (double)(sqrtf(s1) * UP) + ce[5] * err + TINY;
+        err = ce[2] * (double)(sqrtf(s2) * UP) + ce[6] * err + TINY;
+        err = ce[3] * (double)(sqrtf(s3) * UP) + ce[7] * err + TINY;
+        delta += err;
+      }
+      stage_end();
+    };
+    for (int e = 0; e + 1 < E; ++e) network(e, std::false_type{});
+    network(E - 1, std::true_type{});
+    q = cur;
+
+    {
+      const double S = __shfl(total, lane & 15);
+      const double D = __shfl(delta, lane & 15) * (1.0 + 9.5367431640625e-7);
+      if (m_sample) {
+        const double Tt = (double)E * thr;
+        const double slack =
+            8.8817841970012523e-16 * (fabs(S) + D + fabs(Tt));
+        const bool yes = S - D - slack > Tt;
+        const bool no = S + D + slack < Tt;
+        bool ok = inside_e[0];
+        if (need[0]) ok = yes;
+        const bool und = need[0] && !yes && !no;
+        const unsigned char flags =
+            (acc_outer[0] ? 1 : 0) | ((acc_outer[0] && ok) ? 2 : 0);
+        if (valid[0] && lg == 0) a.out_u8[pt[0]] = flags;
+        const unsigned long long ub = __ballot(und && lg == 0);
+        if (und && lg == 0)
+          my_seg[n_und + __popcll(ub & ((1ull << lane) - 1ull))] = (int)pt[0];
+        n_und += __popcll(ub);
+      } else if (valid[0] && lg == 0) {
+        a.out_f64[2 * pt[0]] = S;
+        a.out_f64[2 * pt[0] + 1] = D;
+      }
+    }
+  }
+  if (m_sample && lane == 0) a.seg_count[blockIdx.x * NW + wave] = n_und;
+  if (a.counters != nullptr && lane == 0) {
+    atomicAdd(&a.counters[1], cnt_ell);
+    atomicAdd(&a.counters[3], cnt_scr);
+  }
+}
+
+__global__ void __launch_bounds__(64) screen_compact_kernel(
+    const int* seg, const int* seg_count, long long seg_cap, int n_segs,
+    int* dense, int* totals) {
+  const int s = blockIdx.x, lane = threadIdx.x;
+  int before = 0;
+  for (int i = lane; i < s; i += 64) before += seg_count[i];
+#pragma unroll
+  for (int d = 32; d >= 1; d >>= 1) before += __shfl_xor(before, d);
+  const int mine = seg_count[s];
+  const int* src = seg + (long long)s * seg_cap;
+  for (int i = lane; i < mine; i += 64) dense[before + i] = src[i];
+  if (s == n_segs - 1 && lane == 0) totals[0] = before + mine;
+}
+
+template <int DT, int KT1>
+int launch_screen(const ScreenArgs& a, int blocks, hipStream_t stream) {
+  const size_t lds = (size_t)2 * SCR_REGION * sizeof(double);
+  static bool configured = false;
+  if (!configured) {
+    const hipError_t e = hipFuncSetAttribute(
+        (const void*)nb_screen_kernel<DT, KT1>,
+        hipFuncAttributeMaxDynamicSharedMemorySize, (int)lds);
+    if (e != hipSuccess) {
+      nb_set_error("hipFuncSetAttribute(%zu bytes LDS) failed: %s", lds,
+                   hipGetErrorString(e));
+      return NB_ERR_HIP;
+    }
+    configured = true;
+  }
+  hipLaunchKernelGGL((nb_screen_kernel<DT, KT1>), dim3((unsigned)blocks),
+                     dim3(512), lds, stream, a);
+  return NB_OK;
+}
+
+int screen_blocks(long long n) {
+  const long long n_super = (n + 127) / 128;
+  return (int)(n_super < SCR_BLOCKS ? n_super : SCR_BLOCKS);
+}
+
+long long screen_seg_cap(long long n) {
+  const long long n_super = (n + 127) / 128;
+  const int blocks = screen_blocks(n);
+  return blocks > 0 ? (n_super + blocks - 1) / blocks * 16 : 0;
+}
+
+}
+
+unsigned long long* nb_eval_counters();
+
+long long nb_screen_work_bytes(long long n) {
+  if (n <= 0) return 0;
+  return (long long)sizeof(int) *
+         (4 + SCR_SEGS + SCR_SEGS * screen_seg_cap(n) + n);
+}
+
+int nb_launch_screen(const double* blob_dev, int n_dim, bool sample,
+                     const double* x, long long n, unsigned char* out_u8,
+                     double* out_f64, int* work, int** dense_out,
+                     int** totals_out, hipStream_t stream) {
+  if (n <= 0) return NB_OK;
+  const int blocks = screen_blocks(n);
+  ScreenArgs a = {};
+  a.blob = blob_dev; a.sample = sample ? 1 : 0; a.x = (const nb_gd*)x; a.n = n;
+  a.out_u8 = out_u8; a.out_f64 = out_f64;
+  a.counters = nb_eval_counters();
+  int* totals = work;
+  int* dense = nullptr;
+  if (sample) {
+    a.seg_count = work + 4;
+    a.seg = a.seg_count + SCR_SEGS;
+    a.seg_cap = screen_seg_cap(n);
+    dense = a.seg + SCR_SEGS * a.seg_cap;
+  }
+  const int dt = (n_dim + 15) / 16, kt1 = (n_dim + 1 + 15) / 16;
+  int rc = NB_ERR_UNSUPPORTED;
+  switch (4 * dt + (kt1 - dt)) {
+    case 4: rc = launch_screen<1, 1>(a, blocks, stream); break;
+    case 5: rc = launch_screen<1, 2>(a, blocks, stream); break;
+    case 8: rc = launch_screen<2, 2>(a, blocks, stream); break;
+    case 9: rc = launch_screen<2, 3>(a, blocks, stream); break;
+    case 12: rc = launch_screen<3, 3>(a, blocks, stream); break;
+    case 13: rc = launch_screen<3, 4>(a, blocks, stream); break;
+    case 16: rc = launch_screen<4, 4>(a, blocks, stream); break;
+    case 17: rc = launch_screen<4, 5>(a, blocks, stream); break;
+    case 20: rc = launch_screen<5, 5>(a, blocks, stream); break;
+    case 21: rc = launch_screen<5, 6>(a, blocks, stream); break;
+    case 24: rc = launch_screen<6, 6>(a, blocks, stream); break;
+    case 25: rc = launch_screen<6, 7>(a, blocks, stream); break;
+    case 28: rc = launch_screen<7, 7>(a, blocks, stream); break;
+    case 29: rc = launch_screen<7, 8>(a, blocks, stream); break;
+    case 32: rc = launch_screen<8, 8>(a, blocks, stream); break;
+    case 33: rc = launch_screen<8, 9>(a, blocks, stream); break;
+    default:
+      nb_set_error("nb_launch_screen: n_dim=%d not eligible", n_dim);
+      return NB_ERR_UNSUPPORTED;
+  }
+  if (rc != NB_OK) return rc;
+  NB_HIP_CHECK(hipGetLastError());
+  if (sample) {
+    const int n_segs = blocks * SCR_NW;
+    hipLaunchKernelGGL(screen_compact_kernel, dim3((unsigned)n_segs), dim3(64),
+                       0, stream, a.seg, a.seg_count, a.seg_cap, n_segs, dense,
+                       totals);
+    NB_HIP_CHECK(hipGetLastError());
+    *dense_out = dense;
+    *totals_out = totals;
+  }
+  return NB_OK;
+}
diff --git a/nautilus_amd/device.py b/nautilus_amd/device.py
--- a/nautilus_amd/device.py
+++ b/nautilus_amd/device.py
@@ -102,6 +102,8 @@
         self.thresholds = [float(src.get('score_predict_min', 0.0)) - 1e-9
                            for src in neural]
         self.dense_need = None
+        self.screen = os.environ.get('NB_SCREEN', '1') not in ('0', '')
+        self.undecided_share = None
         for nd, src in zip(n_arr, neural):
             fill_member(nd.ellipsoid, src['ellipsoid'])
             nd.score_predict_min = float(src.get('score_predict_min', 0.0))
@@ -214,6 +216,8 @@
                     self.n_networks >= 1)
         if fused_ok and self.dense_need is not None and self.dense_need > 0.5:
             flags = _buffer('accept', (x.shape[0],), torch.uint8, reuse)
+            if self.screen:
+                return self._accept_screened(seed, offset, x, flags)
             _lib.check(self._lib.nb_accept(self._h, seed, offset, _ptr(x),
                                            x.shape[0], _ptr(flags),
                                            _stream()))
@@ -234,6 +238,30 @@
                 torch.int32)
             self.dense_need = float(totals.sum()) / max(1, n)
         return flags
+
+    def _accept_screened(self, seed, offset, x, flags):
+        n = x.shape[0]
+        need = self._lib.nb_accept_screened_work_bytes(self._h, n)
+        work = _buffer('screen_work', (need,), torch.uint8, True)
+        off = C.c_int64(0)
+        _lib.check(self._lib.nb_accept_screened(
+            self._h, seed, offset, _ptr(x), n, _ptr(flags), _ptr(work), need,
+            C.byref(off), _stream()))
+        DISPATCHES['nb_screen_kernel'] += 1
+        DISPATCHES['nb_eval_fast_kernel'] += 1
+        if self.undecided_share is None and n > 0:
+            und = int(work[off.value:off.value + 4].view(torch.int32)[0])
+            self.undecided_share = und / n
+            if self.undecided_share > SCREEN_MAX_UNDECIDED:
+                self.screen = False
+        return flags
+
+    def screen_score(self, x):
+        x = as_device_points(x, self.n_dim)
+        out = torch.empty((x.shape[0], 2), dtype=torch.float64, device='cuda')
+        _lib.check(self._lib.nb_screen_score(self._h, _ptr(x), x.shape[0],
+                                             _ptr(out), _stream()))
+        return out[:, 0], out[:, 1]
 
     def sample_launch(self, seed, offset, n_draw, mask=2, reuse=False,
                       out_role='compact'):
@@ -313,7 +341,9 @@
 GEOM_ANY, GEOM_FIRST, GEOM_SAMPLE = 0, 1, 2
 NO_BOUND = 2**31 - 1
 WORK_BYTES = 256 << 20
-DISPATCHES = dict(nb_eval_fast_kernel=0, nb_cand_kernel=0)
+DISPATCHES = dict(nb_eval_fast_kernel=0, nb_cand_kernel=0, nb_screen_kernel=0)
+
+SCREEN_MAX_UNDECIDED = 0.25
 GS_OUTER, GS_INSIDE = 1, 2
 
 
@@ -704,7 +734,8 @@
     def read(self):
         c = self.buf.cpu().numpy()
         return dict(outer_point_evals=int(c[0]), ellipsoid_point_evals=int(c[1]),
-                    emulator_point_evals=int(c[2]))
+                    emulator_point_evals=int(c[2]),
+                    screened_point_evals=int(c[3]))
 
 
 class KernelTimer:
```
